# zixunh/vipe

Measured on AMD Instinct MI355X. Metric: dense-BA+flow update iters/s, 512x384 48-KF graph, higher is better.
Workload: dtype f16 (correlation, GRU; fp32 accumulate) + f32 geometry/BA (fp64 reduced system)

## Files before the change

### include/vipe_amd.h

```cpp
#ifndef VIPE_AMD_H
#define VIPE_AMD_H

#include <stdint.h>

#ifdef __cplusplus
extern "C" {
#endif

#define VIPE_F16 0
#define VIPE_F32 1
#define VIPE_F64 2
#define VIPE_U8 3

#define VIPE_OK 0
#define VIPE_EINVAL (-1)
#define VIPE_ENOSPACE (-2)
#define VIPE_EUNSUPPORTED (-3)

#define VIPE_PYRAMID_REFERENCE 0
#define VIPE_PYRAMID_BLOCKED 1

#define VIPE_CAM_PINHOLE 0
#define VIPE_CAM_MEI 1
#define VIPE_CAM_PANORAMA 2

const char* vipe_amd_version(void);
int vipe_amd_abi_version(void);


int vipe_corr_index_forward(const void* d_volume, const float* d_coords, void* d_corr, int B, int h1, int w1,
                            int h2, int w2, int radius, int dtype, void* stream);

int vipe_corr_index_backward(const float* d_coords, const void* d_corr_grad, void* d_volume_grad, int B, int h1,
                             int w1, int h2, int w2, int radius, int dtype, void* stream);

int vipe_corr_pyramid_lookup(const void* const* h_levels, const float* d_coords, void* d_out, int B, int h1, int w1,
                             int h2, int w2, int num_levels, int radius, int dtype, void* stream);

int vipe_corr_pyramid_lookup_nhwc(const void* const* h_levels, const float* d_coords, void* d_out, int B, int h1,
                                  int w1, int h2, int w2, int num_levels, int radius, int dtype, int channel_stride,
                                  void* stream);

int vipe_corr_lookup_conv1x1(const void* const* h_levels, const float* d_coords, const void* d_w_packed,
                             const float* d_bias, void* d_out, int out_ctot, int out_coff, int B, int h1, int w1,
                             int h2, int w2, int Cout, int act, const int* d_slots, int layout, void* stream);

int vipe_corr_pyramid_build(const void* d_fmap1, const void* d_fmap2, void* const* h_levels, int B, int C, int h,
                            int w, int num_levels, void* stream);

int vipe_corr_pyramid_build_indexed(const void* d_fmaps, const int64_t* d_idx1, const int64_t* d_idx2,
                                    const int* d_slots, void* const* h_levels, int B, int C, int h, int w,
                                    int num_levels, int layout, void* stream);

int vipe_corr_blocked_dims(int h, int w, int* dims6);
int64_t vipe_corr_prep_halves(int C, int h, int w);
int vipe_corr_prep(const void* d_fmaps, void* d_prep, int n, int C, int h, int w, void* stream);
int vipe_corr_pyramid_build_prepared(const void* d_prep, int64_t frame_base, int64_t n_prepared, const int64_t* d_idx1, const int64_t* d_idx2,
                                     const int* d_slots, void* const* h_levels, int B, int C, int h, int w, int num_levels,
                                     void* stream);

int vipe_corr_volume(const void* d_fmap1, const void* d_fmap2, void* d_volume, int B, int C, int P, int dtype, void* stream);
int vipe_avg_pool2x2(const void* d_x, void* d_y, int64_t n, int h, int w, int dtype, void* stream);

int vipe_altcorr_forward(const void* d_fmap1, const void* d_fmap2, const float* d_coords, void* d_corr, int B,
                         int H1, int W1, int H2, int W2, int N, int C, int radius, int dtype, void* stream);

int vipe_altcorr_backward(const float* d_fmap1, const float* d_fmap2, const float* d_coords,
                          const float* d_corr_grad, float* d_fmap1_grad, float* d_fmap2_grad, int B, int H1, int W1,
                          int H2, int W2, int N, int C, int radius, void* stream);

int vipe_lie_expm(int group_id, const void* a, void* X, int64_t n, int dtype, int on_device, void* stream);
int vipe_lie_logm(int group_id, const void* X, void* a, int64_t n, int dtype, int on_device, void* stream);
int vipe_lie_inv(int group_id, const void* X, void* Y, int64_t n, int dtype, int on_device, void* stream);
int vipe_lie_mul(int group_id, const void* X, const void* Y, void* Z, int64_t n, int dtype, int on_device,
                 void* stream);
int vipe_lie_adj(int group_id, const void* X, const void* a, void* b, int64_t n, int dtype, int on_device,
                 void* stream);
int vipe_lie_adjT(int group_id, const void* X, const void* a, void* b, int64_t n, int dtype, int on_device,
                  void* stream);
int vipe_lie_act(int group_id, const void* X, const void* p, void* q, int64_t n, int dtype, int on_device,
                 void* stream);
int vipe_lie_act4(int group_id, const void* X, const void* p, void* q, int64_t n, int dtype, int on_device,
                  void* stream);
int vipe_lie_as_matrix(int group_id, const void* X, void* T, int64_t n, int dtype, int on_device,
                       void* stream);
int vipe_lie_projector(int group_id, const void* X, void* P, int64_t n, int dtype, int on_device,
                       void* stream);
int vipe_lie_jinv(int group_id, const void* X, const void* a, void* b, int64_t n, int dtype, int on_device,
                  void* stream);
int vipe_frontend_next_frame(float* d_poses, float* d_disps, int t1, int n_views, int P, int n_mean, int init_pose,
                             void* stream);
int vipe_lie_adjT_bcast(int group_id, const void* X, const void* a, void* b, int64_t n_elem, int64_t rows_per_elem,
                        int dtype, void* stream);
int vipe_lie_act4_bcast(int group_id, const void* X, const void* p, void* q, int64_t n_elem, int64_t rows_per_elem,
                        int dtype, void* stream);
int vipe_lie_expm_backward(int group_id, const void* grad, const void* a, void* da, int64_t n, int dtype,
                           int on_device, void* stream);
int vipe_lie_logm_backward(int group_id, const void* grad, const void* X, void* dX, int64_t n, int dtype,
                           int on_device, void* stream);
int vipe_lie_inv_backward(int group_id, const void* grad, const void* X, void* dX, int64_t n, int dtype,
                          int on_device, void* stream);
int vipe_lie_mul_backward(int group_id, const void* grad, const void* X, const void* Y, void* dX, void* dY,
                          int64_t n, int dtype, int on_device, void* stream);
int vipe_lie_adj_backward(int group_id, const void* grad, const void* X, const void* a, void* dX, void* da,
                          int64_t n, int dtype, int on_device, void* stream);
int vipe_lie_adjT_backward(int group_id, const void* grad, const void* X, const void* a, void* dX, void* da,
                           int64_t n, int dtype, int on_device, void* stream);
int vipe_lie_act_backward(int group_id, const void* grad, const void* X, const void* p, void* dX, void* dp,
                          int64_t n, int dtype, int on_device, void* stream);
int vipe_lie_act4_backward(int group_id, const void* grad, const void* X, const void* p, void* dX, void* dp,
                           int64_t n, int dtype, int on_device, void* stream);


int vipe_reproject(const float* d_poses, const float* d_disps, const float* d_intrinsics, const float* d_rig,
                   const int64_t* d_pi, const int64_t* d_qi, const int64_t* d_pj, const int64_t* d_qj,
                   const int64_t* d_di, float* d_coords, float* d_valid, int M, int ht, int wd, int n_views,
                   int camera, float intr_factor, void* stream);

int vipe_reproject_motion(const float* d_poses, const float* d_disps, const float* d_intrinsics, const float* d_rig,
                          const int64_t* d_pi, const int64_t* d_qi, const int64_t* d_pj, const int64_t* d_qj,
                          const int64_t* d_di, const float* d_target, float* d_coords, void* d_motn, int M, int ht,
                          int wd, int n_views, int camera, float intr_factor, int motn_dtype, void* stream);
int vipe_reproject_motion_nhwc(const float* d_poses, const float* d_disps, const float* d_intrinsics,
                               const float* d_rig, const int64_t* d_pi, const int64_t* d_qi, const int64_t* d_pj,
                               const int64_t* d_qj, const int64_t* d_di, const float* d_target, float* d_coords,
                               void* d_motn, int M, int ht, int wd, int n_views, int camera, float intr_factor,
                               void* stream);

typedef int (*vipe_overlap_fn)(void* user, int piece, int n_pieces, void* stream);

typedef struct {
  int n_poses;
  int n_views;
  int ht, wd;
  int M;
  int t0, t1;
  int n_iters;
  float pose_damping, pose_ep;
  int motion_only;
  int limited_disp;
  int optimize_intrinsics;
  int optimize_rig_rotation;
  int camera;
  float alpha;
  float weight_scale;
  float intr_factor;
  int reuse_plan;
  int path_hint;
  void* overlap_stream;
  vipe_overlap_fn overlap_fn;
  void* overlap_user;
  int solver_options;
  void* profile_ev0;
  void* profile_ev1;
  int profile_iter;
} vipe_ba_params;
#define VIPE_BA_OPT_ONE_CHAIN 1
#define VIPE_BA_OPT_GENERAL_ACCUMULATE 2

int64_t vipe_dense_ba_workspace_bytes(const vipe_ba_params* p);
int vipe_dense_ba(const vipe_ba_params* p, float* d_poses, float* d_disps, const float* d_disps_sens,
                  float* d_intrinsics, float* d_rig, const float* d_target, const float* d_weight,
                  const float* d_disp_damping, const int64_t* d_pi, const int64_t* d_qi, const int64_t* d_pj,
                  const int64_t* d_qj, const int64_t* d_di, void* d_workspace, int64_t workspace_bytes,
                  int* d_info, void* stream);

int vipe_dense_ba_linearize(const vipe_ba_params* p, const float* d_poses, const float* d_disps, const float* d_disps_sens,
                            const float* d_intrinsics, const float* d_rig, const float* d_target, const float* d_weight,
                            const float* d_disp_damping, const int64_t* d_pi, const int64_t* d_qi, const int64_t* d_pj,
                            const int64_t* d_qj, const int64_t* d_di, void* d_workspace, int64_t workspace_bytes,
                            double* d_S_out, int ld_out, int* d_info, void* stream);
int vipe_dense_ba_marginals(const vipe_ba_params* p, void* d_workspace, const double* d_Sinv, int ld, float* d_disp_var,
                            double* d_pose_cov, void* stream);

int64_t vipe_ba_workspace_bytes(int n_poses, int ht, int wd, int E);
int vipe_ba(float* d_poses, float* d_disps, const float* d_intrinsics, const float* d_disps_sens,
            const float* d_targets, const float* d_weights, const float* d_eta, const int64_t* d_ii,
            const int64_t* d_jj, int n_poses, int ht, int wd, int E, int n_eta, int t0, int t1, int iterations,
            float lm, float ep, int motion_only, float* d_dx, float* d_dz, void* d_workspace,
            int64_t workspace_bytes, void* stream);

int vipe_frame_distance(const float* d_poses, const float* d_disps, const float* d_intrinsics, const int64_t* d_pi,
                        const int64_t* d_pj, const int64_t* d_qi, const int64_t* d_qj, const int64_t* d_di,
                        float* d_dist, int M, int ht, int wd, float beta, void* stream);

int vipe_frame_distance_rig(const float* d_poses, const float* d_rig, const float* d_disps, const float* d_intrinsics,
                            int intr_dim, float intr_factor, const int64_t* d_pi, const int64_t* d_qi, const int64_t* d_pj,
                            const int64_t* d_qj, float* d_dist, int M, int n_views, int ht, int wd, float beta,
                            int bidirectional, void* stream);

int vipe_depth_filter(const float* d_poses, const float* d_disps, const float* d_intrinsics, const int64_t* d_inds,
                      const float* d_thresh, float* d_counter, int n, int num, int ht, int wd, void* stream);

int vipe_frame_distance_sphere(const float* d_poses, const float* d_rig, const float* d_disps, const int64_t* d_pi,
                               const int64_t* d_qi, const int64_t* d_pj, const int64_t* d_qj, float* d_dist, int M,
                               int n_views, int ht, int wd, float beta, int bidirectional, void* stream);
int vipe_depth_filter_sphere(const float* d_poses, const float* d_disps, const int64_t* d_inds, const float* d_thresh,
                             float* d_counter, int n, int num, int ht, int wd, void* stream);
int vipe_iproj_sphere(const float* d_poses, const float* d_disps, float* d_points, int n, int ht, int wd, void* stream);

int vipe_projmap(const float* d_poses, const float* d_disps, const float* d_intrinsics, const int64_t* d_ii,
                 const int64_t* d_jj, float* d_coords, float* d_valid, int E, int ht, int wd, void* stream);

int vipe_iproj(const float* d_poses, const float* d_disps, const float* d_intrinsics, float* d_points, int n, int ht,
               int wd, void* stream);

int vipe_scatter(const void* d_src, const int64_t* d_index, void* d_out, int64_t* d_arg_out, int64_t outer,
                 int64_t src_dim, int64_t inner, int64_t out_dim, int reduce, int dtype, void* stream);
int vipe_scatter_rows(const void* d_src, const int64_t* d_index, void* d_out, int64_t* d_arg_out, int64_t outer,
                      int64_t src_dim, int64_t inner, int64_t out_dim, int reduce, int dtype, void* stream);

int vipe_scatter_host(const void* h_src, const int64_t* h_index, void* h_out, int64_t* h_arg_out, int64_t outer,
                      int64_t src_dim, int64_t inner, int64_t out_dim, int reduce, int dtype);

int vipe_scatter_mean_rows_f16(const void* d_src, const int64_t* d_ix, void* d_out, int E, int n_out, int64_t inner,
                               void* stream);

int vipe_segment_mean_nhwc_f16(const void* d_src, int src_ctot, int src_coff, const int* d_order, const int* d_rowptr,
                               void* d_out, int n_out, int64_t rows_per_item, int C, void* stream);

int vipe_corr_sampler_forward(const void* d_in1, const void* d_in2, void* d_out, int B, int C, int H, int W, int kH,
                              int kW, int patchH, int patchW, int padH, int padW, int dilH, int dilW,
                              int dil_patchH, int dil_patchW, int dH, int dW, int dtype, void* stream);
int vipe_corr_sampler_backward(const void* d_in1, const void* d_in2, const void* d_grad_out, void* d_grad1,
                               void* d_grad2, int B, int C, int H, int W, int kH, int kW, int patchH, int patchW,
                               int padH, int padW, int dilH, int dilW, int dil_patchH, int dil_patchW, int dH,
                               int dW, int dtype, void* stream);

int vipe_corr_sampler_forward_host(const float* h_in1, const float* h_in2, float* h_out, int B, int C, int H, int W, int kH,
                                   int kW, int patchH, int patchW, int padH, int padW, int dilH, int dilW, int dil_patchH,
                                   int dil_patchW, int dH, int dW);
int vipe_corr_sampler_backward_host(const float* h_in1, const float* h_in2, const float* h_grad_out, float* h_grad1,
                                    float* h_grad2, int B, int C, int H, int W, int kH, int kW, int patchH, int patchW,
                                    int padH, int padW, int dilH, int dilW, int dil_patchH, int dil_patchW, int dH, int dW);

int vipe_nearest_neighbours(const float* d_query, int qdim, const float* d_tree, int tdim, int64_t M, int64_t N, int knn,
                            float* d_dist, int* d_idx, void* stream);

int vipe_ms_deform_attn_forward(const void* d_value, const int64_t* d_spatial_shapes, const int64_t* d_level_start_index,
                                const void* d_sampling_loc, const void* d_attn_weight, void* d_output, int64_t bs,
                                int64_t Lv, int heads, int C, int L, int64_t Lq, int P, int dtype, void* stream);
int vipe_ms_deform_attn_backward(const void* d_value, const int64_t* d_spatial_shapes, const int64_t* d_level_start_index,
                                 const void* d_sampling_loc, const void* d_attn_weight, const void* d_grad_output,
                                 void* d_grad_value, void* d_grad_sampling_loc, void* d_grad_attn_weight, int64_t bs,
                                 int64_t Lv, int heads, int C, int L, int64_t Lq, int P, int dtype, void* stream);

#define VIPE_ACT_NONE 0
#define VIPE_ACT_RELU 1
#define VIPE_ACT_SIGMOID 2
#define VIPE_ACT_TANH 3
int vipe_conv_pack_weights(const void* d_w_oihw, void* d_w_packed, int Cout, int Cin, int KH, int KW, int src_dtype,
                           void* stream);
int vipe_conv2d_nhwc_f16(const void* d_x, const void* d_w_packed, const float* d_bias, const float* d_extra,
                         void* d_y, int B, int H, int W, int Cin, int cin_total, int cin_off, int Cout,
                         int cout_total, int cout_off, int KH, int KW, int act, void* stream);

int vipe_conv_packed_dims(int Cout, int Cin, int KH, int KW, int* cout_pad, int* cin_pad, int* k_pad);

#define VIPE_CONV_PARTIAL 6
#define VIPE_CONV_ACCINIT_F32 0x100
int vipe_conv2d_fused(const void* d_x0, int x0_ctot, int x0_coff, const void* d_x1, int x1_ctot, int x1_coff,
                      int split, const void* d_w_packed, const float* d_bias, const float* d_extra, int extra_stride,
                      int extra_off, void* d_y, int y_ctot, int y_coff, void* d_y2, int y2_ctot, int y2_coff,
                      const void* d_net, int net_ctot, int net_coff, const void* d_z, float* d_fout,
                      const void* d_accinit, int ai_ctot, int ai_coff, int B, int H, int W, int Cin, int Cout, int KH,
                      int KW, int act, int mode, void* stream);

typedef struct {
  const void *corr0_w, *corr2_w, *flow0_w, *flow2_w, *gw_w, *zr_w, *q_w, *zr_s_w, *q_s_w, *heads0_w, *heads2_w, *agg2_w, *eta_w;
  const void *zr_n_w, *zr_x_w;
  const float *corr0_b, *corr2_b, *flow0_b, *flow2_b, *gw_b, *zr_b, *q_b, *heads0_b, *heads2_b, *agg2_b, *eta_b;
  const float* glo_wT;
  const float* glo_b;
} vipe_update_weights;
typedef struct {
  int E, H, W, n_src;
  const void* levels[4];
  const float* coords;
  const int* slots;
  int h2, w2, pyramid_layout;
  const void* corr;
  const void* motn;
  const void* net;
  void* net_out;
  void* xbuf;
  const void* pgate;
  void *c1, *f1, *zb, *rnet;
  void* hbuf;
  float* dw;
  float *glo, *extra;
  const int *order, *rowptr;
  void *agg, *a2;
  float* eta;
  void* side_stream;
  float* pzr;
  int gate_state;
} vipe_update_buffers;
int vipe_update_operator(const vipe_update_weights* weights, const vipe_update_buffers* buffers, void* stream);

int vipe_update_gate_state(const vipe_update_weights* weights, const vipe_update_buffers* buffers, const void* d_net,
                           int parts, void* stream);
typedef struct {
  const vipe_update_weights* weights;
  const vipe_update_buffers* buffers;
  const void* net;
  const int* bounds;
  int n_bounds;
} vipe_gate_state_job;
int vipe_update_gate_state_piece(void* user, int piece, int n_pieces, void* stream);

int vipe_glo_context(const float* d_glo_sum, const float* d_wT, const float* d_bias, float* d_extra, int E, int hw,
                     void* stream);

typedef struct {
  const void* src;
  void* dst;
  const int64_t* idx;
  int64_t src_row_pitch, dst_row_pitch;
  int64_t seg_bytes, seg_pitch;
  int n_seg;
  int n_rows;
  int dst_row0;
} vipe_rows_job;
int vipe_rows_gather(const vipe_rows_job* jobs, int n_jobs, void* stream);
typedef struct {
  const void* src;
  const int64_t* frame;
  void* dst;
  int64_t dst_row_pitch;
  int dst_ctot, dst_coff;
  int dst_row0;
} vipe_nhwc_job;
int vipe_gather_nchw_to_nhwc_f16(const vipe_nhwc_job* jobs, int n_jobs, int n_rows, int C, int P, void* stream);

int vipe_flow_score(const float* d_dw, const unsigned char* d_invalid, float* d_score, int n_views, int P, void* stream);

int vipe_update_finish(const float* d_coords1, const float* d_dw, const unsigned char* d_mask, float* d_target,
                       float* d_weight, const float* d_eta, const int64_t* d_du, float* d_damping, int E, int n_src, int ht,
                       int wd, void* stream);

int vipe_enc_prep(const float* d_img, void* d_x4, int V, int H, int W, void* stream);
int vipe_enc_stem(const void* d_x4, const void* d_w, const float* d_bias, void* d_y, float* d_out_stats, int B, int H,
                  int W, int relu, void* stream);
int vipe_enc_conv(const void* d_x, const float* d_in_stats, const void* d_w, const float* d_bias, const void* d_res,
                  void* d_y, float* d_out_stats, int B, int H, int W, int Cin, int Cout, int ksize, int stride,
                  int relu, int nchw, int tanh_split, void* stream);
int vipe_enc_finish(const void* d_raw, const float* d_raw_stats, const void* d_res, const float* d_res_stats,
                    void* d_out, int B, int HW, int C, void* stream);

int vipe_frame_ingest(const void* d_rgb, int rgb_dtype, const unsigned char* d_mask, const float* d_depth, int H0, int W0,
                      int h1, int w1, int top, int left, int H, int W, float* d_images, void* d_x4,
                      unsigned char* d_mask8, float* d_disps_sens, void* stream);

int vipe_convex_upsample(const void* d_mask, int mask_dtype, const float* d_data, float* d_out, const int64_t* d_rows,
                         int N, int R, int h, int w, int C, void* stream);

#define VIPE_KLT_OOB 1
#define VIPE_KLT_LOW_TEXTURE 2
#define VIPE_KLT_RESIDUAL 4
#define VIPE_KLT_FB 8
#define VIPE_KLT_MASKED 16
#define VIPE_KLT_DIVERGED 32

int vipe_klt_pyramid(const void* d_rgb, int rgb_dtype, int H, int W, int L, float* d_pyr, void* stream);

int vipe_klt_detect(const float* d_img, int H, int W, const unsigned char* d_mask, const unsigned char* d_cell_busy,
                    int cell, int border, float min_eig, float* d_out, void* stream);

int vipe_klt_track(const float* d_pyr_a, const float* d_pyr_b, int H, int W, int L, const float* d_pts, int N,
                   const float* d_fb_ref, const unsigned char* d_mask, int win_radius, int n_iters, float eps, int border,
                   float min_eig, float max_residual, float fb_thresh, float max_flow, int cell, float* d_out,
                   unsigned char* d_status, float* d_resid, unsigned char* d_cell_busy, void* stream);

#ifdef __cplusplus
}
#endif
#endif
```

### vipe_amd/csrc/conv_mfma.hip

```cpp
#include <stdlib.h>

#include <type_traits>

#include "common.cuh"

namespace {

typedef _Float16 half8 __attribute__((ext_vector_type(8)));
typedef _Float16 half4 __attribute__((ext_vector_type(4)));
typedef float float16v __attribute__((ext_vector_type(16)));
typedef float float4v __attribute__((ext_vector_type(4)));

enum Epi { EPI_PLAIN = 0, EPI_GLO = 1, EPI_ZR = 2, EPI_Q = 3, EPI_HEADS = 4, EPI_ETA = 5, EPI_PARTIAL = 6 };

struct ConvArgs {
  const half_t* x0; int x0_ctot, x0_coff;
  const half_t* x1; int x1_ctot, x1_coff;
  int split;
  const half_t* w;
  const float* bias;
  const float* extra;
  int extra_stride, extra_off;
  half_t* y; int y_ctot, y_coff;
  int B, H, W, Cin, Cin_pad, Cout, Cout_pad, KH, KW, nsteps;
  int act, epi;
  const half_t* net; int net_ctot, net_coff;
  const half_t* zbuf;
  half_t* y2; int y2_ctot, y2_coff;
  float* fout;
  const half_t* accinit; int ai_ctot, ai_coff;
  int ai_f32;
  int f_wp, f_hwp, f_tiles, f_pieces, f_xbytes, f_p1lo, f_p1hi;
  unsigned f_magic;
};

constexpr int BNP = 128;
constexpr int BK = 64;

__device__ __forceinline__ int swz(int row, int k8) { return row * 128 + ((k8 ^ ((row >> 1) & 7)) << 4); }

__device__ __forceinline__ float act_apply(float v, int act) {
  switch (act) {
    case VIPE_ACT_RELU: return fmaxf(v, 0.0f);
    case VIPE_ACT_SIGMOID: return 1.0f / (1.0f + __expf(-v));
    case VIPE_ACT_TANH: return tanhf(v);
    default: return v;
  }
}

template <int BMC, int WAVES_M, int WAVES_N, bool SMALLCIN>
__global__ __launch_bounds__(256) void conv_mfma_kernel(ConvArgs a) {
  constexpr int TM = BMC / (WAVES_M * 32);
  constexpr int TN = BNP / (WAVES_N * 32);
  static_assert(WAVES_M * WAVES_N == 4, "4 waves");
  constexpr int W_ITEMS = BMC * 8 / 256;
  constexpr int X_ITEMS = BNP * 8 / 256;

  extern __shared__ __align__(16) unsigned char lds[];
  unsigned char* ldsW = lds;
  unsigned char* ldsX = lds + 2 * BMC * 128;

  const int tid = threadIdx.x, lane = tid & 63, wave = tid >> 6;
  const int wm = wave / WAVES_N, wn = wave % WAVES_N;
  const int64_t M = (int64_t)a.B * a.H * a.W;
  const int64_t pix0 = (int64_t)blockIdx.x * BNP;
  const int cout0 = blockIdx.y * BMC;
  const int HW = a.H * a.W;

  const int k8 = tid & 7;
  int xe[X_ITEMS], xy[X_ITEMS], xx[X_ITEMS];
  bool xvalid[X_ITEMS];
#pragma unroll
  for (int j = 0; j < X_ITEMS; ++j) {
    const int64_t m = pix0 + (tid >> 3) + 32 * j;
    xvalid[j] = m < M;
    const int64_t mm = xvalid[j] ? m : 0;
    xe[j] = (int)(mm / HW);
    const int rem = (int)(mm % HW);
    xy[j] = rem / a.W;
    xx[j] = rem % a.W;
  }
  const int ph = a.KH / 2, pw = a.KW / 2;
  const int csteps = a.Cin_pad / BK;

  half8 wreg[W_ITEMS], xreg[X_ITEMS];

  auto issue_loads = [&](int s) {
    const half_t* wb = a.w + ((int64_t)s * a.Cout_pad + cout0) * BK;
#pragma unroll
    for (int j = 0; j < W_ITEMS; ++j) {
      const int row = (tid >> 3) + 32 * j;
      wreg[j] = *reinterpret_cast<const half8*>(wb + row * BK + k8 * 8);
    }
    if constexpr (!SMALLCIN) {
      const int tap = s / csteps, c0 = (s % csteps) * BK;
      const int dy = tap / a.KW - ph, dx = tap % a.KW - pw;
      const int c = c0 + k8 * 8;
      const bool cok = c < a.Cin;
      const bool s0 = c < a.split;
      const half_t* src = s0 ? a.x0 : a.x1;
      const int ctot = s0 ? a.x0_ctot : a.x1_ctot;
      const int coff = s0 ? a.x0_coff + c : a.x1_coff + (c - a.split);
#pragma unroll
      for (int j = 0; j < X_ITEMS; ++j) {
        const int yy = xy[j] + dy, xc = xx[j] + dx;
        const bool ok = cok & xvalid[j] & (yy >= 0) & (yy < a.H) & (xc >= 0) & (xc < a.W);
        half8 v = {0, 0, 0, 0, 0, 0, 0, 0};
        if (ok) v = *reinterpret_cast<const half8*>(src + ((int64_t)(xe[j] * a.H + yy) * a.W + xc) * ctot + coff);
        xreg[j] = v;
      }
    } else {
      const int q = s * 8 + k8;
#pragma unroll
      for (int j = 0; j < X_ITEMS; ++j) {
        half4 lo = {0, 0, 0, 0}, hi = {0, 0, 0, 0};
#pragma unroll
        for (int h = 0; h < 2; ++h) {
          const int tap = 2 * q + h;
          if (tap < a.KH * a.KW) {
            const int yy = xy[j] + tap / a.KW - ph, xc = xx[j] + tap % a.KW - pw;
            if (xvalid[j] & (yy >= 0) & (yy < a.H) & (xc >= 0) & (xc < a.W)) {
              const half4 v = *reinterpret_cast<const half4*>(
                  a.x0 + ((int64_t)(xe[j] * a.H + yy) * a.W + xc) * a.x0_ctot + a.x0_coff);
              if (h == 0) lo = v; else hi = v;
            }
          }
        }
        xreg[j] = half8{lo[0], lo[1], lo[2], lo[3], hi[0], hi[1], hi[2], hi[3]};
      }
    }
  };
  auto write_lds = [&](int buf) {
#pragma unroll
    for (int j = 0; j < W_ITEMS; ++j) {
      const int row = (tid >> 3) + 32 * j;
      *reinterpret_cast<half8*>(ldsW + buf * BMC * 128 + swz(row, k8)) = wreg[j];
    }
#pragma unroll
    for (int j = 0; j < X_ITEMS; ++j) {
      const int row = (tid >> 3) + 32 * j;
      *reinterpret_cast<half8*>(ldsX + buf * BNP * 128 + swz(row, k8)) = xreg[j];
    }
  };

  float16v acc[TM][TN];
#pragma unroll
  for (int i = 0; i < TM; ++i)
#pragma unroll
    for (int j = 0; j < TN; ++j)
#pragma unroll
      for (int r = 0; r < 16; ++r) acc[i][j][r] = 0.0f;

  issue_loads(0);
  write_lds(0);
  __syncthreads();
  const int lrow = lane & 31, lhalf = lane >> 5;
  for (int s = 0; s < a.nsteps; ++s) {
    const int cur = s & 1;
    if (s + 1 < a.nsteps) issue_loads(s + 1);
    const unsigned char* bw = ldsW + cur * BMC * 128;
    const unsigned char* bx = ldsX + cur * BNP * 128;
#pragma unroll
    for (int kk = 0; kk < BK / 16; ++kk) {
      half8 wf[TM], xf[TN];
#pragma unroll
      for (int i = 0; i < TM; ++i)
        wf[i] = *reinterpret_cast<const half8*>(bw + swz((wm * TM + i) * 32 + lrow, kk * 2 + lhalf));
#pragma unroll
      for (int j = 0; j < TN; ++j)
        xf[j] = *reinterpret_cast<const half8*>(bx + swz((wn * TN + j) * 32 + lrow, kk * 2 + lhalf));
#pragma unroll
      for (int i = 0; i < TM; ++i)
#pragma unroll
        for (int j = 0; j < TN; ++j)
          acc[i][j] = __builtin_amdgcn_mfma_f32_32x32x16_f16(wf[i], xf[j], acc[i][j], 0, 0, 0);
    }
    if (s + 1 < a.nsteps) write_lds(cur ^ 1);
    __syncthreads();
  }

#include "conv_epilogue.inc"
}

__device__ __attribute__((aligned(16))) unsigned char g_zero_page[64];

__device__ __forceinline__ void glds16(const void* g, unsigned lds_addr) {
#if defined(__HIP_DEVICE_COMPILE__)
  unsigned keep;
  const unsigned base = __builtin_amdgcn_readfirstlane(lds_addr);
  asm volatile(
      "s_mov_b32 %0, m0\n\ts_mov_b32 m0, %2\n\ts_nop 0\n\tglobal_load_lds_dwordx4 %1, off\n\ts_mov_b32 m0, %0"
      : "=&s"(keep)
      : "v"(g), "s"(base)
      : "memory");
#endif
}

__device__ __forceinline__ unsigned lds_address(const void* p) {
  return (unsigned)(uintptr_t)(__attribute__((address_space(3))) const unsigned char*)p;
}

template <int BMC, int WAVES_M, int WAVES_N>
__global__ __launch_bounds__(256) void conv_mfma_glds_kernel(ConvArgs a, int gy) {
  constexpr int TM = BMC / (WAVES_M * 32);
  constexpr int TN = BNP / (WAVES_N * 32);
  static_assert(WAVES_M * WAVES_N == 4, "4 waves");
  constexpr int WP = BMC / 32;
  constexpr int XP = BNP / 32;

  extern __shared__ __align__(16) unsigned char lds[];
  unsigned char* ldsW = lds;
  unsigned char* ldsX = lds + 2 * BMC * 128;

  const int tid = threadIdx.x, lane = tid & 63, wave = __builtin_amdgcn_readfirstlane(tid >> 6);
  const int wm = wave / WAVES_N, wn = wave % WAVES_N;
  const int nb = gridDim.x;
  const int L = xcd_remap(blockIdx.x, nb);
  const int64_t M = (int64_t)a.B * a.H * a.W;
  const int64_t pix0 = (int64_t)(L / gy) * BNP;
  const int cout0 = (L % gy) * BMC;
  const int HW = a.H * a.W;
  const int ph = a.KH / 2, pw = a.KW / 2;
  const int csteps = a.Cin_pad / BK;
  const int r8 = lane >> 3, sl = lane & 7;

  int woff[WP];
#pragma unroll
  for (int q = 0; q < WP; ++q) {
    const int row = (wave * WP + q) * 8 + r8;
    woff[q] = row * BK + ((sl ^ ((row >> 1) & 7)) << 3);
  }
  const half_t* xb0[XP];
  const half_t* xb1[XP];
  int xk8[XP], py[XP], px[XP];
  unsigned xmask[XP];
#pragma unroll
  for (int q = 0; q < XP; ++q) {
    const int row = (wave * XP + q) * 8 + r8;
    const int64_t m = pix0 + row;
    const bool ok = m < M;
    const int64_t mm = ok ? m : 0;
    const int rem = (int)(mm % HW);
    py[q] = ok ? rem / a.W : -100000;
    px[q] = rem % a.W;
    const int k8 = sl ^ ((row >> 1) & 7);
    xk8[q] = k8 * 8;
    xb0[q] = a.x0 + mm * a.x0_ctot + a.x0_coff + k8 * 8;
    xb1[q] = a.x1 + mm * a.x1_ctot + a.x1_coff + k8 * 8 - a.split;
    xmask[q] = 0;
  }
  for (int t = 0; t < a.KH * a.KW; ++t) {
    const int dy = t / a.KW - ph, dx = t % a.KW - pw;
#pragma unroll
    for (int q = 0; q < XP; ++q) {
      const int yy = py[q] + dy, xc = px[q] + dx;
      if (yy >= 0 && yy < a.H && xc >= 0 && xc < a.W) xmask[q] |= 1u << t;
    }
  }
  const half_t* zp = reinterpret_cast<const half_t*>(g_zero_page);

  auto issue = [&](int s, int buf) {
    const half_t* wb = a.w + ((int64_t)s * a.Cout_pad + cout0) * BK;
    unsigned char* lw = ldsW + buf * BMC * 128 + wave * WP * 1024;
#pragma unroll
    for (int q = 0; q < WP; ++q)
      glds16(wb + woff[q], lds_address(lw) + q * 1024);
    const int tap = s / csteps, c0 = (s % csteps) * BK;
    const int dy = tap / a.KW - ph, dx = tap % a.KW - pw;
    const bool s0 = c0 < a.split;
    const int64_t delta = (int64_t)(dy * a.W + dx) * (s0 ? a.x0_ctot : a.x1_ctot) + c0;
    const int crem = a.Cin - c0;
    unsigned char* lx = ldsX + buf * BNP * 128 + wave * XP * 1024;
#pragma unroll
    for (int q = 0; q < XP; ++q) {
      const bool ok = ((xmask[q] >> tap) & 1u) && (xk8[q] < crem);
      const half_t* p = (s0 ? xb0[q] : xb1[q]) + delta;
      glds16(ok ? p : zp, lds_address(lx) + q * 1024);
    }
  };

  float16v acc[TM][TN];
#pragma unroll
  for (int i = 0; i < TM; ++i)
#pragma unroll
    for (int j = 0; j < TN; ++j)
#pragma unroll
      for (int r = 0; r < 16; ++r) acc[i][j][r] = 0.0f;

  issue(0, 0);
  asm volatile("s_waitcnt vmcnt(0)" ::: "memory");
  __syncthreads();
  const int lrow = lane & 31, lhalf = lane >> 5;
  for (int s = 0; s < a.nsteps; ++s) {
    const int cur = s & 1;
    const unsigned char* bw = ldsW + cur * BMC * 128;
    const unsigned char* bx = ldsX + cur * BNP * 128;
    half8 wf[BK / 16][TM], xf[BK / 16][TN];
#pragma unroll
    for (int kk = 0; kk < BK / 16; ++kk) {
#pragma unroll
      for (int i = 0; i < TM; ++i)
        wf[kk][i] = *reinterpret_cast<const half8*>(bw + swz((wm * TM + i) * 32 + lrow, kk * 2 + lhalf));
#pragma unroll
      for (int j = 0; j < TN; ++j)
        xf[kk][j] = *reinterpret_cast<const half8*>(bx + swz((wn * TN + j) * 32 + lrow, kk * 2 + lhalf));
    }
    __builtin_amdgcn_sched_barrier(0);
    if (s + 1 < a.nsteps) issue(s + 1, cur ^ 1);
    __builtin_amdgcn_sched_barrier(0);
#pragma unroll
    for (int kk = 0; kk < BK / 16; ++kk)
#pragma unroll
      for (int i = 0; i < TM; ++i)
#pragma unroll
        for (int j = 0; j < TN; ++j)
          acc[i][j] = __builtin_amdgcn_mfma_f32_32x32x16_f16(wf[kk][i], xf[kk][j], acc[i][j], 0, 0, 0);
    asm volatile("s_waitcnt vmcnt(0)" ::: "memory");
    __syncthreads();
  }
#include "conv_epilogue.inc"
}

constexpr int HALO_TH = 4, HALO_TW = 64;
constexpr int HALO_PITCH = HALO_TW + 2;
constexpr int HALO_ROWS = (HALO_TH + 2) * HALO_PITCH;

__device__ __forceinline__ void glds16_off(const void* base, unsigned voff_bytes, unsigned lds_addr) {
#if defined(__HIP_DEVICE_COMPILE__)
  unsigned keep;
  const unsigned lb = __builtin_amdgcn_readfirstlane(lds_addr);
  const uint64_t bu = (uint64_t)base;
  const uint64_t bs = ((uint64_t)(unsigned)__builtin_amdgcn_readfirstlane((int)(bu >> 32)) << 32) |
                      (unsigned)__builtin_amdgcn_readfirstlane((int)bu);
  asm volatile(
      "s_mov_b32 %0, m0\n\ts_mov_b32 m0, %3\n\ts_nop 0\n\tglobal_load_lds_dwordx4 %1, %2\n\ts_mov_b32 m0, %0"
      : "=&s"(keep)
      : "v"(voff_bytes), "s"(bs), "s"(lb)
      : "memory");
#endif
}

__device__ __forceinline__ uint64_t uniform64(uint64_t v) {
  return ((uint64_t)(unsigned)__builtin_amdgcn_readfirstlane((int)(v >> 32)) << 32) | (unsigned)__builtin_amdgcn_readfirstlane((int)v);
}
__device__ __forceinline__ void dma16s(uint64_t sbase, unsigned voff_bytes, unsigned lds_addr) {
#if defined(__HIP_DEVICE_COMPILE__)
  unsigned keep;
  asm volatile("s_mov_b32 %0, m0\n\ts_mov_b32 m0, %3\n\ts_nop 0\n\tglobal_load_lds_dwordx4 %1, %2\n\ts_mov_b32 m0, %0"
               : "=&s"(keep)
               : "v"(voff_bytes), "s"(sbase), "s"(lds_addr)
               : "memory");
#endif
}
__device__ __forceinline__ void dma16v(uint64_t lane_ptr, unsigned lds_addr) {
#if defined(__HIP_DEVICE_COMPILE__)
  unsigned keep;
  asm volatile("s_mov_b32 %0, m0\n\ts_mov_b32 m0, %2\n\ts_nop 0\n\tglobal_load_lds_dwordx4 %1, off\n\ts_mov_b32 m0, %0"
               : "=&s"(keep)
               : "v"(lane_ptr), "s"(lds_addr)
               : "memory");
#endif
}

constexpr int H32_PIECES = (HALO_ROWS + 15) / 16;
constexpr int H32_XBYTES = H32_PIECES * 1024;
constexpr int H32_XP = (H32_PIECES + 7) / 8;
constexpr int H32_BK = 32;

__device__ __forceinline__ int swzf(int row) { return ((row >> 2) & 1) << 1; }
__device__ __forceinline__ int swz32(int row, int c) { return row * 64 + ((c ^ swzf(row)) << 4); }


__device__ __forceinline__ int flat_pixel(int q, int e, int H, int W, int wp, int hwp, unsigned magic) {
  if ((unsigned)q >= (unsigned)hwp) return -1;
  const int y = (int)__umulhi((unsigned)q, magic);
  const int x = q - y * wp;
  return x < W ? (e * H + y) * W + x : -1;
}

template <int BMC, int KS, bool M16, int VAR = 0, bool FLAT = false>
__global__ __launch_bounds__(512) __attribute__((amdgpu_waves_per_eu(4, 4))) void conv_halo32_kernel(ConvArgs a, int gy) {
  static_assert(M16, "only the 16x16x32 form exists");
  constexpr int MI = BMC >= 128 ? 4 : 2, NJ = BMC == 32 ? 2 : 4;
  constexpr int BP = HALO_TH * HALO_TW;
  constexpr int WSTAGE = BMC * 64;
  extern __shared__ __align__(16) unsigned char lds[];

  const int tid = threadIdx.x, lane = tid & 63, wave = __builtin_amdgcn_readfirstlane(tid >> 6);
  const int wm = BMC == 32 ? 0 : (wave >> 2), wn = wave & 3;
  const int pxh = BMC == 32 ? (wave >> 2) * 32 : 0;
  const int L = xcd_remap(blockIdx.x, gridDim.x);
  const int tile = L / gy, cout0 = (L % gy) * BMC;
  const int xsegs = a.W / HALO_TW, tiles_per_img = FLAT ? a.f_tiles : (a.H / HALO_TH) * xsegs;
  const int e = tile / tiles_per_img, trem = tile % tiles_per_img;
  const int y0 = (trem / xsegs) * HALO_TH, x0 = (trem % xsegs) * HALO_TW;
  const int q0 = trem * BP;
  const int pitch = FLAT ? a.f_wp : HALO_PITCH;
  const int xbytes = FLAT ? a.f_xbytes : H32_XBYTES;
  const int npieces = FLAT ? a.f_pieces : H32_PIECES;
  auto pix_of = [&](int pl) -> int64_t {
    if constexpr (FLAT) return flat_pixel(q0 + pl, e, a.H, a.W, a.f_wp, a.f_hwp, a.f_magic);
    else return ((int64_t)(e * a.H + y0 + (pl >> 6))) * a.W + x0 + (pl & 63);
  };
  const int cs32 = a.Cin_pad / H32_BK, cs64 = a.Cin_pad / 64;
  const int r16 = lane >> 2, sl = lane & 3;

  const unsigned ldsW_a = lds_address(lds), ldsX_a = ldsW_a + 3 * WSTAGE;
  const unsigned sink_a = ldsX_a + 2 * xbytes;
  const unsigned char* ldsW = lds;
  const unsigned char* ldsX = lds + 3 * WSTAGE;
  const half_t* zp = reinterpret_cast<const half_t*>(g_zero_page);

  constexpr int WPIECES = BMC / 16;
  const bool wreal = wave < WPIECES;
  const int wrow = (wave % WPIECES) * 16 + r16;
  const unsigned woff = (unsigned)(wrow * 64 + ((sl ^ swzf(wrow)) << 3)) * 2u;
  const unsigned wdst = ldsW_a + (wave % WPIECES) * 1024;
  int xpix[FLAT ? 1 : H32_XP];
  const int xk = (sl ^ swzf(r16)) * 8;
  if constexpr (!FLAT) {
#pragma unroll
    for (int i = 0; i < H32_XP; ++i) {
      const int pce = wave + 8 * i;
      const int r = pce * 16 + r16;
      const int hy = r / HALO_PITCH, hx = r % HALO_PITCH;
      const int y = y0 + hy - 1, x = x0 + hx - 1;
      const bool ok = pce < H32_PIECES && r < HALO_ROWS && y >= 0 && y < a.H && x >= 0 && x < a.W;
      xpix[i] = ok ? (e * a.H + y) * a.W + x : -1;
    }
  }
  auto piece_used = [&](int i) {
    const int pce = wave + 8 * i;
    if constexpr (FLAT) return pce < npieces && (KS == 3 || (pce >= a.f_p1lo && pce <= a.f_p1hi));
    else return pce < H32_PIECES && (KS == 3 || (pce >= 4 && pce <= 20));
  };
  auto issueX = [&](int c, int i, int buf) {
    const int c0 = c * H32_BK;
    const bool s0 = c0 < a.split;
    const int ctot = s0 ? a.x0_ctot : a.x1_ctot;
    const int cb = (s0 ? a.x0_coff : a.x1_coff - a.split) + c0;
    int xp;
    if constexpr (FLAT) xp = flat_pixel(q0 - pitch - 1 + (wave + 8 * i) * 16 + r16, e, a.H, a.W, a.f_wp, a.f_hwp, a.f_magic);
    else xp = xpix[i];
    const bool ok = xp >= 0 && (c0 + xk < a.Cin);
    const uint64_t off = ((uint64_t)(unsigned)xp * (unsigned)ctot + (unsigned)(cb + xk)) * 2u;
    const char* src = reinterpret_cast<const char*>(s0 ? a.x0 : a.x1) + off;
    glds16(ok ? (const void*)src : (const void*)zp, ldsX_a + buf * xbytes + (wave + 8 * i) * 1024);
  };
  auto wsrc = [&](int tap, int c) {
    return a.w + ((int64_t)(tap * cs64 + (c >> 1)) * a.Cout_pad + cout0) * BK + (c & 1) * H32_BK;
  };
  auto issueW = [&](const half_t* wb, int slot) {
    if (wreal) glds16_off(wb, woff, wdst + slot * WSTAGE);
    else glds16(zp, sink_a);
  };
  const uint64_t zp64 = uniform64((uint64_t)zp);
  const uint64_t wbase = uniform64((uint64_t)(a.w + (int64_t)cout0 * BK));
  const unsigned tstride = (unsigned)cs64 * (unsigned)a.Cout_pad * BK * 2u;
  const unsigned sink_u = __builtin_amdgcn_readfirstlane(sink_a), wdst_u = __builtin_amdgcn_readfirstlane(wdst);
  const unsigned ldsX_u = __builtin_amdgcn_readfirstlane(ldsX_a + wave * 1024);
  auto issueW2 = [&](int tap, int c, int slot, bool more_) {
    const unsigned off = (unsigned)tap * tstride + ((unsigned)(c >> 1) * (unsigned)a.Cout_pad * BK + (unsigned)(c & 1) * H32_BK) * 2u;
    const bool on = more_ && wreal;
    dma16s(on ? wbase + off : zp64, on ? woff : 0u, on ? wdst_u + slot * WSTAGE : sink_u);
  };
  auto issueX2 = [&](int c, int i, int buf, bool on) {
    const int c0 = c * H32_BK;
    const bool s0 = c0 < a.split;
    const int ctot = s0 ? a.x0_ctot : a.x1_ctot;
    const int cb = (s0 ? a.x0_coff : a.x1_coff - a.split) + c0;
    int xp;
    if constexpr (FLAT) xp = flat_pixel(q0 - pitch - 1 + (wave + 8 * i) * 16 + r16, e, a.H, a.W, a.f_wp, a.f_hwp, a.f_magic);
    else xp = xpix[i];
    const bool ok = on && xp >= 0 && (c0 + xk < a.Cin);
    const uint64_t off = ((uint64_t)(unsigned)xp * (unsigned)ctot + (unsigned)(cb + xk)) * 2u;
    const uint64_t base = (uint64_t)(s0 ? a.x0 : a.x1);
    dma16v(ok ? base + off : zp64, on ? ldsX_u + buf * xbytes + i * 8192 : sink_u);
  };

  float4v acc16[MI][NJ];
#pragma unroll
  for (int i = 0; i < MI; ++i)
#pragma unroll
    for (int j = 0; j < NJ; ++j) acc16[i][j] = float4v{0.0f, 0.0f, 0.0f, 0.0f};
  if constexpr (BMC >= 64) {
    if (a.accinit) {
#pragma unroll
      for (int j = 0; j < NJ; ++j) {
        const int64_t m = pix_of(wn * 64 + j * 16 + (lane & 15));
        if (FLAT && m < 0) continue;
#pragma unroll
        for (int i = 0; i < MI; ++i) {
          const int cg = cout0 + wm * (MI * 16) + i * 16 + 4 * (lane >> 4);
          if constexpr (VAR == 1) {
            const float4 v = *reinterpret_cast<const float4*>(reinterpret_cast<const float*>(a.accinit) + m * a.ai_ctot +
                                                              a.ai_coff + cg);
            acc16[i][j] = float4v{v.x, v.y, v.z, v.w};
          } else {
            const half4 v = *reinterpret_cast<const half4*>(a.accinit + m * a.ai_ctot + a.ai_coff + cg);
            acc16[i][j] = float4v{(float)v[0], (float)v[1], (float)v[2], (float)v[3]};
          }
        }
      }
    }
  }

  const int l16 = lane & 15, lk = lane >> 4;
  const int wa0 = swz32(wm * MI * 16 + l16, lk);
  const int Rl0 = (FLAT ? wn * HALO_TW : wn * HALO_PITCH) + pxh + l16;
  auto mma_step = [&](const unsigned char* bw, const unsigned char* bx, int Rl, int dy, int dx) {
    const int rb = Rl + (dy + 1) * pitch + (dx + 1);
    const int xa0 = swz32(rb, lk);
    half8 wf[MI];
#pragma unroll
    for (int i = 0; i < MI; ++i) wf[i] = *reinterpret_cast<const half8*>(bw + (wa0 + i * 1024));
#pragma unroll
    for (int j = 0; j < NJ; ++j) {
      const half8 xf = *reinterpret_cast<const half8*>(bx + (xa0 + j * 1024));
#pragma unroll
      for (int i = 0; i < MI; ++i)
        acc16[i][j] = __builtin_amdgcn_mfma_f32_16x16x32_f16(wf[i], xf, acc16[i][j], 0, 0, 0);
    }
  };

  auto load_frags = [&](const unsigned char* bw, const unsigned char* bx, int Rl, int dy, int dx, half8 (&wf)[MI], half8 (&xf)[NJ]) {
    const int xa0 = swz32(Rl + (dy + 1) * pitch + (dx + 1), lk);
#pragma unroll
    for (int i = 0; i < MI; ++i) wf[i] = *reinterpret_cast<const half8*>(bw + (wa0 + i * 1024));
#pragma unroll
    for (int j = 0; j < NJ; ++j) xf[j] = *reinterpret_cast<const half8*>(bx + (xa0 + j * 1024));
  };
  auto mma_frags = [&](const half8 (&wf)[MI], const half8 (&xf)[NJ]) {
#pragma unroll
    for (int j = 0; j < NJ; ++j)
#pragma unroll
      for (int i = 0; i < MI; ++i) acc16[i][j] = __builtin_amdgcn_mfma_f32_16x16x32_f16(wf[i], xf[j], acc16[i][j], 0, 0, 0);
  };

#pragma unroll
  for (int i = 0; i < H32_XP; ++i)
    if (piece_used(i)) issueX(0, i, 0);
  issueW(wsrc(0, 0), 0);
  if constexpr (KS == 3) issueW(wsrc(1, 0), 1);
  asm volatile("s_waitcnt vmcnt(0)" ::: "memory");
  __syncthreads();

  if constexpr (KS == 3) {
    for (int c = 0; c < cs32; ++c) {
      const unsigned char* bx = ldsX + (c & 1) * xbytes;
      const bool more = c + 1 < cs32;
      int Rl = Rl0;
      asm volatile("" : "+v"(Rl));
      auto tap_step = [&](auto TAPC) {
        constexpr int TAP = decltype(TAPC)::value;
        constexpr int T2 = TAP + 2;
        half8 wf[MI], xf[NJ];
        load_frags(ldsW + (TAP % 3) * WSTAGE, bx, Rl, TAP / 3 - 1, TAP % 3 - 1, wf, xf);
        if constexpr (T2 < 9) issueW2(T2, c, T2 % 3, true);
        else issueW2(T2 - 9, c + 1, T2 % 3, more);
        if constexpr (TAP < H32_XP) issueX2(c + 1, TAP, (c + 1) & 1, more && piece_used(TAP));
        mma_frags(wf, xf);
        if constexpr (TAP == 0 || TAP == 4) asm volatile("s_waitcnt vmcnt(2)" ::: "memory");
        else if constexpr (TAP < 4) asm volatile("s_waitcnt vmcnt(3)" ::: "memory");
        else asm volatile("s_waitcnt vmcnt(1)" ::: "memory");
        __syncthreads();
      };
      tap_step(std::integral_constant<int, 0>{});
      tap_step(std::integral_constant<int, 1>{});
      tap_step(std::integral_constant<int, 2>{});
      tap_step(std::integral_constant<int, 3>{});
      tap_step(std::integral_constant<int, 4>{});
      tap_step(std::integral_constant<int, 5>{});
      tap_step(std::integral_constant<int, 6>{});
      tap_step(std::integral_constant<int, 7>{});
      tap_step(std::integral_constant<int, 8>{});
    }
  } else {
    for (int c = 0; c < cs32; ++c) {
      const unsigned char* bx = ldsX + (c & 1) * xbytes;
      if (c + 1 < cs32) {
        issueW(wsrc(0, c + 1), (c + 1) & 1);
#pragma unroll
        for (int i = 0; i < H32_XP; ++i)
          if (piece_used(i)) issueX(c + 1, i, (c + 1) & 1);
      }
      mma_step(ldsW + (c & 1) * WSTAGE, bx, Rl0, 0, 0);
      asm volatile("s_waitcnt vmcnt(0)" ::: "memory");
      __syncthreads();
    }
  }
  asm volatile("s_waitcnt vmcnt(0)" ::: "memory");
  __syncthreads();

  constexpr int CPP = BMC / 8;
  constexpr int NIT = BP * CPP / 512, PSTEP = 512 / CPP;
  const int ch = (tid % CPP) * 8, co = cout0 + ch, pl0 = tid / CPP;
  if constexpr (BMC >= 64) {
    if constexpr (VAR == 2) {
      {
#pragma unroll
        for (int j = 0; j < NJ; ++j) {
          const int64_t m = pix_of(wn * 64 + j * 16 + l16);
          if (FLAT && m < 0) continue;
#pragma unroll
          for (int i = 0; i < MI; ++i) {
            const int cg = cout0 + wm * (MI * 16) + i * 16 + 4 * lk;
            if (cg + 4 <= a.Cout)
              *reinterpret_cast<float4*>(a.fout + m * a.y_ctot + a.y_coff + cg) =
                  make_float4(acc16[i][j][0], acc16[i][j][1], acc16[i][j][2], acc16[i][j][3]);
          }
        }
        return;
      }
    }
    constexpr int PITCH = BMC + 8;
    half_t* stage = reinterpret_cast<half_t*>(lds);
    auto stage_all = [&](auto ACTC) {
      constexpr int ACT = decltype(ACTC)::value;
      auto put = [&](int cl, int pl, float4 b, float v0, float v1, float v2, float v3) {
        half4 h;
        h[0] = (half_t)act_apply(v0 + b.x, ACT);
        h[1] = (half_t)act_apply(v1 + b.y, ACT);
        h[2] = (half_t)act_apply(v2 + b.z, ACT);
        h[3] = (half_t)act_apply(v3 + b.w, ACT);
        *reinterpret_cast<half4*>(stage + pl * PITCH + cl) = h;
      };
      auto bias4 = [&](int cl) {
        const int cg = cout0 + cl;
        float4 b = *reinterpret_cast<const float4*>(a.bias + cg);
        if (a.extra && cg + 4 <= a.Cout) {
          const float4 x = *reinterpret_cast<const float4*>(a.extra + (int64_t)e * a.extra_stride + a.extra_off + cg);
          b.x += x.x; b.y += x.y; b.z += x.z; b.w += x.w;
        }
        return b;
      };
#pragma unroll
      for (int i = 0; i < MI; ++i) {
        const int cl = wm * (MI * 16) + i * 16 + 4 * lk;
        const float4 b = bias4(cl);
#pragma unroll
        for (int j = 0; j < NJ; ++j)
          put(cl, wn * 64 + j * 16 + l16, b, acc16[i][j][0], acc16[i][j][1], acc16[i][j][2], acc16[i][j][3]);
      }
    };
    const int actsel = a.epi == EPI_PLAIN ? a.act : (a.epi == EPI_Q ? VIPE_ACT_TANH : VIPE_ACT_SIGMOID);
    if (actsel == VIPE_ACT_RELU) stage_all(std::integral_constant<int, VIPE_ACT_RELU>{});
    else if (actsel == VIPE_ACT_SIGMOID) stage_all(std::integral_constant<int, VIPE_ACT_SIGMOID>{});
    else if (actsel == VIPE_ACT_TANH) stage_all(std::integral_constant<int, VIPE_ACT_TANH>{});
    else stage_all(std::integral_constant<int, VIPE_ACT_NONE>{});
    const bool want_net = a.epi == EPI_GLO || a.epi == EPI_Q || (a.epi == EPI_ZR && co >= 128);
    const bool want_z = a.epi == EPI_Q;
    half8 nvv[NIT], zvv[NIT];
    {
      const int cn = a.epi == EPI_ZR ? co - 128 : co;
#pragma unroll
      for (int it = 0; it < NIT; ++it) {
        const int64_t m = pix_of(pl0 + PSTEP * it);
        if (FLAT && m < 0) continue;
        if (want_net) nvv[it] = *reinterpret_cast<const half8*>(a.net + m * a.net_ctot + a.net_coff + cn);
        if (want_z) zvv[it] = *reinterpret_cast<const half8*>(a.zbuf + m * 128 + co);
      }
    }
    __syncthreads();
    float gsum[8] = {0, 0, 0, 0, 0, 0, 0, 0};
#pragma unroll
    for (int it = 0; it < NIT; ++it) {
      const int pl = pl0 + PSTEP * it;
      const int64_t m = pix_of(pl);
      if (FLAT && m < 0) continue;
      const half8 sv = *reinterpret_cast<const half8*>(stage + pl * PITCH + ch);
      half8 o = sv;
      half_t* dst = nullptr;
      if (a.epi == EPI_PLAIN) {
        dst = a.y + m * a.y_ctot + a.y_coff + co;
      } else if (a.epi == EPI_GLO) {
#pragma unroll
        for (int q = 0; q < 8; ++q) gsum[q] += (float)sv[q] * (float)nvv[it][q];
      } else if (a.epi == EPI_ZR) {
        if (co < 128) {
          dst = a.y + m * a.y_ctot + a.y_coff + co;
        } else {
#pragma unroll
          for (int q = 0; q < 8; ++q) o[q] = (half_t)((float)sv[q] * (float)nvv[it][q]);
          dst = a.y2 + m * a.y2_ctot + a.y2_coff + co - 128;
        }
      } else if (a.epi == EPI_Q) {
#pragma unroll
        for (int q = 0; q < 8; ++q) {
          const float z = (float)zvv[it][q];
          o[q] = (half_t)((1.0f - z) * (float)nvv[it][q] + z * (float)sv[q]);
        }
        dst = a.y + m * a.y_ctot + a.y_coff + co;
      }
      if (dst) {
        if (co + 8 <= a.Cout) {
          *reinterpret_cast<half8*>(dst) = o;
        } else {
          for (int q = 0; q < 8 && co + q < a.Cout; ++q) dst[q] = o[q];
        }
      }
    }
    if (a.epi == EPI_GLO) {
      float* red = reinterpret_cast<float*>(lds);
      __syncthreads();
#pragma unroll
      for (int q = 0; q < 8; ++q) red[(tid / CPP) * (BMC + 1) + ch + q] = gsum[q];
      __syncthreads();
      if (tid < BMC) {
        float t = 0.0f;
        for (int r = 0; r < 512 / CPP; ++r) t += red[r * (BMC + 1) + tid];
        if (cout0 + tid < a.Cout) atomicAdd(a.fout + (int64_t)e * a.Cout + cout0 + tid, t);
      }
    }
  } else {
    constexpr int PITCH = BMC + 4;
    float* stage = reinterpret_cast<float*>(lds);
#pragma unroll
    for (int i = 0; i < MI; ++i)
#pragma unroll
      for (int j = 0; j < NJ; ++j)
        *reinterpret_cast<float4*>(stage + (wn * 64 + pxh + j * 16 + l16) * PITCH + i * 16 + 4 * lk) =
            make_float4(acc16[i][j][0], acc16[i][j][1], acc16[i][j][2], acc16[i][j][3]);
    __syncthreads();
    float bv[8];
#pragma unroll
    for (int q = 0; q < 8; ++q) {
      bv[q] = a.bias[co + q];
      if (a.extra && co + q < a.Cout) bv[q] += a.extra[(int64_t)e * a.extra_stride + a.extra_off + co + q];
    }
#pragma unroll
    for (int it = 0; it < NIT; ++it) {
      const int pl = pl0 + PSTEP * it;
      const int64_t m = pix_of(pl);
      if (FLAT && m < 0) continue;
      const float4 v0 = *reinterpret_cast<const float4*>(stage + pl * PITCH + ch);
      const float4 v1 = *reinterpret_cast<const float4*>(stage + pl * PITCH + ch + 4);
      const float v[8] = {v0.x + bv[0], v0.y + bv[1], v0.z + bv[2], v0.w + bv[3],
                          v1.x + bv[4], v1.y + bv[5], v1.z + bv[6], v1.w + bv[7]};
      if (a.epi == EPI_HEADS) {
        if (ch == 0)
          *reinterpret_cast<float4*>(a.fout + m * 4) =
              make_float4((float)(half_t)v[0], (float)(half_t)v[1], (float)(half_t)act_apply(v[2], VIPE_ACT_SIGMOID),
                          (float)(half_t)act_apply(v[3], VIPE_ACT_SIGMOID));
      } else if (a.epi == EPI_ETA) {
        if (ch == 0) {
          const float sp = v[0] > 20.0f ? v[0] : log1pf(__expf(v[0]));
          a.fout[m] = 0.01f * (float)(half_t)sp;
        }
      } else {
        half_t* dst = a.y + m * a.y_ctot + a.y_coff + co;
        half8 o;
#pragma unroll
        for (int q = 0; q < 8; ++q) o[q] = (half_t)act_apply(v[q], a.act);
        if (co + 8 <= a.Cout) {
          *reinterpret_cast<half8*>(dst) = o;
        } else {
          for (int q = 0; q < 8 && co + q < a.Cout; ++q) dst[q] = o[q];
        }
      }
    }
  }
}

constexpr int NRW_WBYTES = 9 * 1024;

template <bool FLAT>
__global__ __launch_bounds__(512) __attribute__((amdgpu_waves_per_eu(4, 4))) void conv_halo32_narrow_kernel(ConvArgs a) {
  extern __shared__ __align__(16) unsigned char lds[];
  const int tid = threadIdx.x, lane = tid & 63, wave = __builtin_amdgcn_readfirstlane(tid >> 6);
  const int wn = wave & 3, pxh = (wave >> 2) * 32;
  const int tile = xcd_remap(blockIdx.x, gridDim.x);
  const int xsegs = a.W / HALO_TW, tiles_per_img = FLAT ? a.f_tiles : (a.H / HALO_TH) * xsegs;
  const int e = tile / tiles_per_img, trem = tile % tiles_per_img;
  const int y0 = (trem / xsegs) * HALO_TH, x0 = (trem % xsegs) * HALO_TW;
  const int q0 = trem * (HALO_TH * HALO_TW);
  const int pitch = FLAT ? a.f_wp : HALO_PITCH, xbytes = FLAT ? a.f_xbytes : H32_XBYTES;
  const int npieces = FLAT ? a.f_pieces : H32_PIECES;
  auto pix_of = [&](int pl) -> int64_t {
    if constexpr (FLAT) return flat_pixel(q0 + pl, e, a.H, a.W, a.f_wp, a.f_hwp, a.f_magic);
    else return ((int64_t)(e * a.H + y0 + (pl >> 6))) * a.W + x0 + (pl & 63);
  };
  const int cs32 = a.Cin_pad / H32_BK, cs64 = a.Cin_pad / 64;
  const int r16 = lane >> 2, sl = lane & 3, l16 = lane & 15, lk = lane >> 4;
  const unsigned ldsW_a = lds_address(lds), ldsX_a = ldsW_a + 2 * NRW_WBYTES;
  const unsigned char* ldsW = lds;
  const unsigned char* ldsX = lds + 2 * NRW_WBYTES;
  const half_t* zp = reinterpret_cast<const half_t*>(g_zero_page);

  int xpix[H32_XP];
  const int xk = (sl ^ swzf(r16)) * 8;
#pragma unroll
  for (int i = 0; i < H32_XP; ++i) {
    const int pce = wave + 8 * i;
    const int r = pce * 16 + r16;
    if constexpr (FLAT) {
      xpix[i] = pce < npieces ? flat_pixel(q0 - pitch - 1 + r, e, a.H, a.W, a.f_wp, a.f_hwp, a.f_magic) : -1;
    } else {
      const int hy = r / HALO_PITCH, hx = r % HALO_PITCH;
      const int y = y0 + hy - 1, x = x0 + hx - 1;
      const bool ok = pce < H32_PIECES && r < HALO_ROWS && y >= 0 && y < a.H && x >= 0 && x < a.W;
      xpix[i] = ok ? (e * a.H + y) * a.W + x : -1;
    }
  }
  auto issue = [&](int c, int buf) {
    const int c0 = c * H32_BK;
    const bool s0 = c0 < a.split;
    const int ctot = s0 ? a.x0_ctot : a.x1_ctot;
    const int cb = (s0 ? a.x0_coff : a.x1_coff - a.split) + c0;
#pragma unroll
    for (int i = 0; i < H32_XP; ++i) {
      if (wave + 8 * i < npieces) {
        const bool ok = xpix[i] >= 0 && (c0 + xk < a.Cin);
        const uint64_t off = ((uint64_t)(unsigned)xpix[i] * (unsigned)ctot + (unsigned)(cb + xk)) * 2u;
        const char* src = reinterpret_cast<const char*>(s0 ? a.x0 : a.x1) + off;
        glds16(ok ? (const void*)src : (const void*)zp, ldsX_a + buf * xbytes + (wave + 8 * i) * 1024);
      }
    }
    const unsigned woff = (unsigned)(r16 * 64 + ((sl ^ swzf(r16)) << 3)) * 2u;
    const half_t* wb = a.w + ((int64_t)(wave * cs64 + (c >> 1)) * a.Cout_pad) * BK + (c & 1) * H32_BK;
    glds16_off(wb, woff, ldsW_a + buf * NRW_WBYTES + wave * 1024);
    if (wave == 0) {
      const half_t* w8 = a.w + ((int64_t)(8 * cs64 + (c >> 1)) * a.Cout_pad) * BK + (c & 1) * H32_BK;
      glds16_off(w8, woff, ldsW_a + buf * NRW_WBYTES + 8 * 1024);
    }
  };

  float4v acc[2] = {float4v{0.f, 0.f, 0.f, 0.f}, float4v{0.f, 0.f, 0.f, 0.f}};
  const int wa0 = swz32(l16, lk);
  const int Rl0 = (FLAT ? wn * HALO_TW : wn * HALO_PITCH) + pxh + l16;
  issue(0, 0);
  asm volatile("s_waitcnt vmcnt(0)" ::: "memory");
  __syncthreads();
  for (int c = 0; c < cs32; ++c) {
    if (c + 1 < cs32) issue(c + 1, (c + 1) & 1);
    const unsigned char* bw = ldsW + (c & 1) * NRW_WBYTES;
    const unsigned char* bx = ldsX + (c & 1) * xbytes;
#pragma unroll
    for (int tap = 0; tap < 9; ++tap) {
      const int rb = Rl0 + (tap / 3) * pitch + (tap % 3);
      const int xa0 = swz32(rb, lk);
      const half8 wf = *reinterpret_cast<const half8*>(bw + (wa0 + tap * 1024));
#pragma unroll
      for (int j = 0; j < 2; ++j) {
        const half8 xf = *reinterpret_cast<const half8*>(bx + (xa0 + j * 1024));
        acc[j] = __builtin_amdgcn_mfma_f32_16x16x32_f16(wf, xf, acc[j], 0, 0, 0);
      }
    }
    asm volatile("s_waitcnt vmcnt(0)" ::: "memory");
    __syncthreads();
  }
  constexpr int PITCH = 20;
  float* stage = reinterpret_cast<float*>(lds);
#pragma unroll
  for (int j = 0; j < 2; ++j)
    *reinterpret_cast<float4*>(stage + (wn * 64 + pxh + j * 16 + l16) * PITCH + 4 * lk) =
        make_float4(acc[j][0], acc[j][1], acc[j][2], acc[j][3]);
  __syncthreads();
  const int64_t m = tid < HALO_TH * HALO_TW ? pix_of(tid) : -1;
  if (tid < HALO_TH * HALO_TW && (!FLAT || m >= 0)) {
    float v[16];
#pragma unroll
    for (int q = 0; q < 4; ++q) {
      const float4 t4 = *reinterpret_cast<const float4*>(stage + tid * PITCH + 4 * q);
      v[4 * q] = t4.x; v[4 * q + 1] = t4.y; v[4 * q + 2] = t4.z; v[4 * q + 3] = t4.w;
    }
#pragma unroll
    for (int q = 0; q < 16; ++q) {
      v[q] += a.bias[q];
      if (a.extra && q < a.Cout) v[q] += a.extra[(int64_t)e * a.extra_stride + a.extra_off + q];
    }
    if (a.epi == EPI_HEADS) {
      *reinterpret_cast<float4*>(a.fout + m * 4) =
          make_float4((float)(half_t)v[0], (float)(half_t)v[1], (float)(half_t)act_apply(v[2], VIPE_ACT_SIGMOID),
                      (float)(half_t)act_apply(v[3], VIPE_ACT_SIGMOID));
    } else if (a.epi == EPI_ETA) {
      const float sp = v[0] > 20.0f ? v[0] : log1pf(__expf(v[0]));
      a.fout[m] = 0.01f * (float)(half_t)sp;
    } else {
      half_t* dst = a.y + m * a.y_ctot + a.y_coff;
      for (int q = 0; q < a.Cout; ++q) dst[q] = (half_t)act_apply(v[q], a.act);
    }
  }
}

constexpr int GLO_PITCH = 136;
constexpr size_t GLO_LDS = 256 * GLO_PITCH * 2 + 128 * 4;

__global__ __launch_bounds__(512) __attribute__((amdgpu_waves_per_eu(4, 4))) void conv1x1_glo_kernel(ConvArgs a) {
  extern __shared__ __align__(16) unsigned char lds[];
  half_t* xt = reinterpret_cast<half_t*>(lds);
  float* gacc = reinterpret_cast<float*>(lds + 256 * GLO_PITCH * 2);
  const int tid = threadIdx.x, lane = tid & 63, wave = tid >> 6;
  const int l16 = lane & 15, kg = lane >> 4;
  const int wq = wave & 3, wp = wave >> 2;
  const int HW = a.H * a.W;
  const int tpi = (HW + 255) / 256;
  const int e = blockIdx.x / tpi, p0 = (blockIdx.x % tpi) * 256;
  const int64_t pix0 = (int64_t)e * HW + p0;
  if (tid < 128) gacc[tid] = 0.0f;
#pragma unroll
  for (int it = 0; it < 8; ++it) {
    const int i = tid + 512 * it, px = i >> 4, ck = i & 15;
    half8 v = {0, 0, 0, 0, 0, 0, 0, 0};
    if (p0 + px < HW) v = *reinterpret_cast<const half8*>(a.x0 + (pix0 + px) * a.x0_ctot + a.x0_coff + ck * 8);
    *reinterpret_cast<half8*>(xt + px * GLO_PITCH + ck * 8) = v;
  }
  half8 af[2][4];
#pragma unroll
  for (int i = 0; i < 2; ++i)
#pragma unroll
    for (int s2 = 0; s2 < 4; ++s2) {
      const int k = 32 * s2 + 8 * kg, r = 32 * wq + 16 * i + l16;
      af[i][s2] = *reinterpret_cast<const half8*>(a.w + ((int64_t)(k >> 6) * a.Cout_pad + r) * 64 + (k & 63));
    }
  float4 bv[2];
#pragma unroll
  for (int i = 0; i < 2; ++i) bv[i] = *reinterpret_cast<const float4*>(a.bias + 32 * wq + 16 * i + 4 * kg);
  __syncthreads();
  float gs[2][4] = {{0, 0, 0, 0}, {0, 0, 0, 0}};
#pragma unroll 2
  for (int j = 0; j < 8; ++j) {
    const int pxb = wp * 128 + j * 16 + l16;
    float4v acc[2] = {float4v{0.f, 0.f, 0.f, 0.f}, float4v{0.f, 0.f, 0.f, 0.f}};
#pragma unroll
    for (int s2 = 0; s2 < 4; ++s2) {
      const half8 xf = *reinterpret_cast<const half8*>(xt + pxb * GLO_PITCH + 32 * s2 + 8 * kg);
#pragma unroll
      for (int i = 0; i < 2; ++i) acc[i] = __builtin_amdgcn_mfma_f32_16x16x32_f16(af[i][s2], xf, acc[i], 0, 0, 0);
    }
#pragma unroll
    for (int i = 0; i < 2; ++i) {
      const half4 nv = *reinterpret_cast<const half4*>(xt + pxb * GLO_PITCH + 32 * wq + 16 * i + 4 * kg);
      const float b4[4] = {bv[i].x, bv[i].y, bv[i].z, bv[i].w};
#pragma unroll
      for (int r = 0; r < 4; ++r)
        gs[i][r] += (float)(half_t)act_apply(acc[i][r] + b4[r], VIPE_ACT_SIGMOID) * (float)nv[r];
    }
  }
#pragma unroll
  for (int i = 0; i < 2; ++i)
#pragma unroll
    for (int r = 0; r < 4; ++r) {
      float v = gs[i][r];
      v += __builtin_bit_cast(float, __builtin_amdgcn_update_dpp(0, __builtin_bit_cast(int, v), 0xB1, 0xf, 0xf, true));
      v += __builtin_bit_cast(float, __builtin_amdgcn_update_dpp(0, __builtin_bit_cast(int, v), 0x4E, 0xf, 0xf, true));
      v += __builtin_bit_cast(float, __builtin_amdgcn_update_dpp(0, __builtin_bit_cast(int, v), 0x141, 0xf, 0xf, true));
      v += __builtin_bit_cast(float, __builtin_amdgcn_update_dpp(0, __builtin_bit_cast(int, v), 0x140, 0xf, 0xf, true));
      if (l16 == 0) atomicAdd(&gacc[32 * wq + 16 * i + 4 * kg + r], v);
    }
  __syncthreads();
  if (tid < a.Cout) atomicAdd(a.fout + (int64_t)e * a.Cout + tid, gacc[tid]);
}

constexpr int C7_PW = HALO_TW + 6, C7_ROWS = HALO_TH + 6;
constexpr int C7_WBYTES = 4 * 128 * 128;
constexpr int C7_XBYTES = ((C7_PW * C7_ROWS * 8 + 15) / 16) * 16;
constexpr int C7_LDS = (C7_WBYTES + C7_XBYTES) > (256 * 136 * 2) ? (C7_WBYTES + C7_XBYTES) : (256 * 136 * 2);

template <bool FLAT>
__global__ __launch_bounds__(512) __attribute__((amdgpu_waves_per_eu(4, 4))) void conv7x7_c4_kernel(ConvArgs a, int gy) {
  extern __shared__ __align__(16) unsigned char lds[];
  const int tid = threadIdx.x, lane = tid & 63, wave = __builtin_amdgcn_readfirstlane(tid >> 6);
  const int wm = wave >> 2, wn = wave & 3;
  const int L = xcd_remap(blockIdx.x, gridDim.x);
  const int tile = L / gy, cout0 = (L % gy) * 128;
  const int xsegs = a.W / HALO_TW, tiles_per_img = FLAT ? a.f_tiles : (a.H / HALO_TH) * xsegs;
  const int e = tile / tiles_per_img, trem = tile % tiles_per_img;
  const int y0 = (trem / xsegs) * HALO_TH, x0 = (trem % xsegs) * HALO_TW;
  const int q0 = trem * (HALO_TH * HALO_TW), pitch = FLAT ? a.f_wp : C7_PW;
  auto pix_of = [&](int pl) -> int64_t {
    if constexpr (FLAT) return flat_pixel(q0 + pl, e, a.H, a.W, a.f_wp, a.f_hwp, a.f_magic);
    else return ((int64_t)(e * a.H + y0 + (pl >> 6))) * a.W + x0 + (pl & 63);
  };
  const int l16 = lane & 15, lk = lane >> 4;
  const unsigned ldsW_a = lds_address(lds);
  unsigned char* ldsX = lds + C7_WBYTES;

  {
    const int r8 = lane >> 3, sl = lane & 7;
#pragma unroll
    for (int q = 0; q < 8; ++q) {
      const int pce = wave * 8 + q;
      const int blk = pce >> 4, row = (pce & 15) * 8 + r8;
      const half_t* src = a.w + ((int64_t)blk * a.Cout_pad + cout0 + row) * 64 + ((sl ^ ((row >> 1) & 7)) << 3);
      glds16(src, ldsW_a + pce * 1024);
    }
  }
  if constexpr (FLAT) {
    const int nh = HALO_TH * HALO_TW + 6 * pitch + 6;
    for (int i = tid; i < nh; i += 512) {
      const int m = flat_pixel(q0 - 3 * pitch - 3 + i, e, a.H, a.W, a.f_wp, a.f_hwp, a.f_magic);
      uint2 v = make_uint2(0u, 0u);
      if (m >= 0) v = *reinterpret_cast<const uint2*>(a.x0 + (int64_t)m * a.x0_ctot + a.x0_coff);
      *reinterpret_cast<uint2*>(ldsX + i * 8) = v;
    }
  } else {
    for (int i = tid; i < C7_PW * C7_ROWS; i += 512) {
      const int hy = i / C7_PW, hx = i % C7_PW;
      const int y = y0 + hy - 3, x = x0 + hx - 3;
      uint2 v = make_uint2(0u, 0u);
      if (y >= 0 && y < a.H && x >= 0 && x < a.W)
        v = *reinterpret_cast<const uint2*>(a.x0 + ((int64_t)(e * a.H + y) * a.W + x) * a.x0_ctot + a.x0_coff);
      *reinterpret_cast<uint2*>(ldsX + i * 8) = v;
    }
  }
  asm volatile("s_waitcnt vmcnt(0)" ::: "memory");
  __syncthreads();

  float4v acc[4][4];
#pragma unroll
  for (int i = 0; i < 4; ++i)
#pragma unroll
    for (int j = 0; j < 4; ++j) acc[i][j] = float4v{0.0f, 0.0f, 0.0f, 0.0f};
#pragma unroll
  for (int st = 0; st < 7; ++st) {
    half8 wf[4];
#pragma unroll
    for (int i = 0; i < 4; ++i)
      wf[i] = *reinterpret_cast<const half8*>(lds + (st >> 1) * 16384 + swz(wm * 64 + i * 16 + l16, (st & 1) * 4 + lk));
    const int t0 = min(st * 8 + lk * 2, 48), t1 = min(st * 8 + lk * 2 + 1, 48);
    const int wrow = FLAT ? wn * HALO_TW : wn * C7_PW;
    const int o0 = (wrow + (t0 / 7) * pitch + l16 + t0 % 7) * 8, o1 = (wrow + (t1 / 7) * pitch + l16 + t1 % 7) * 8;
#pragma unroll
    for (int j = 0; j < 4; ++j) {
      const half4 lo = *reinterpret_cast<const half4*>(ldsX + o0 + j * 128);
      const half4 hi = *reinterpret_cast<const half4*>(ldsX + o1 + j * 128);
      const half8 xf = {lo[0], lo[1], lo[2], lo[3], hi[0], hi[1], hi[2], hi[3]};
#pragma unroll
      for (int i = 0; i < 4; ++i) acc[i][j] = __builtin_amdgcn_mfma_f32_16x16x32_f16(wf[i], xf, acc[i][j], 0, 0, 0);
    }
  }
  __syncthreads();
  constexpr int PITCH = 136;
  half_t* stage = reinterpret_cast<half_t*>(lds);
#pragma unroll
  for (int i = 0; i < 4; ++i) {
    const int cl = wm * 64 + i * 16 + 4 * lk;
    const float4 b = *reinterpret_cast<const float4*>(a.bias + cout0 + cl);
#pragma unroll
    for (int j = 0; j < 4; ++j) {
      half4 h;
      h[0] = (half_t)act_apply(acc[i][j][0] + b.x, a.act);
      h[1] = (half_t)act_apply(acc[i][j][1] + b.y, a.act);
      h[2] = (half_t)act_apply(acc[i][j][2] + b.z, a.act);
      h[3] = (half_t)act_apply(acc[i][j][3] + b.w, a.act);
      *reinterpret_cast<half4*>(stage + (wn * 64 + j * 16 + l16) * PITCH + cl) = h;
    }
  }
  __syncthreads();
  const int ch = (tid & 15) * 8, co = cout0 + ch;
#pragma unroll
  for (int it = 0; it < 8; ++it) {
    const int pl = (tid >> 4) + 32 * it;
    const int64_t m = pix_of(pl);
    if (FLAT && m < 0) continue;
    const half8 o = *reinterpret_cast<const half8*>(stage + pl * PITCH + ch);
    half_t* dst = a.y + m * a.y_ctot + a.y_coff + co;
    if (co + 8 <= a.Cout) {
      *reinterpret_cast<half8*>(dst) = o;
    } else {
      for (int q = 0; q < 8 && co + q < a.Cout; ++q) dst[q] = o[q];
    }
  }
}

__global__ void pack_weights_kernel(const void* __restrict__ src, half_t* __restrict__ dst, int Cout, int Cin, int KH,
                                    int KW, int Cout_pad, int Cin_pad, int K_pad, int src_f32, int smallcin) {
  const int64_t total = (int64_t)K_pad * Cout_pad;
  for (int64_t i = (int64_t)blockIdx.x * blockDim.x + threadIdx.x; i < total; i += (int64_t)gridDim.x * blockDim.x) {
    const int kin = (int)(i % 64);
    const int co = (int)((i / 64) % Cout_pad);
    const int s = (int)(i / (64 * (int64_t)Cout_pad));
    const int k = s * 64 + kin;
    int tap, c;
    if (smallcin) { tap = k / 4; c = k % 4; }
    else { tap = k / Cin_pad; c = k % Cin_pad; }
    float v = 0.0f;
    if (co < Cout && c < Cin && tap < KH * KW) {
      const int64_t o = (((int64_t)co * Cin + c) * KH + tap / KW) * KW + tap % KW;
      v = src_f32 ? reinterpret_cast<const float*>(src)[o] : (float)reinterpret_cast<const half_t*>(src)[o];
    }
    dst[i] = (half_t)v;
  }
}

inline int round_up(int x, int m) { return (x + m - 1) / m * m; }

}


extern "C" {

VIPE_EXPORT int vipe_conv_packed_dims(int Cout, int Cin, int KH, int KW, int* cout_pad, int* cin_pad, int* k_pad) {
  if (Cout <= 0 || Cin <= 0 || KH <= 0 || KW <= 0) return VIPE_EINVAL;
  const int cp = Cout <= 32 ? 32 : (Cout <= 64 ? 64 : round_up(Cout, 128));
  int cinp, kp;
  if (Cin == 4) { cinp = 4; kp = round_up(KH * KW * 4, 64); }
  else { cinp = round_up(Cin, 64); kp = KH * KW * cinp; }
  if (cout_pad) *cout_pad = cp;
  if (cin_pad) *cin_pad = cinp;
  if (k_pad) *k_pad = kp;
  return VIPE_OK;
}

VIPE_EXPORT int vipe_conv_pack_weights(const void* d_w_oihw, void* d_w_packed, int Cout, int Cin, int KH, int KW,
                                       int src_dtype, void* stream) {
  VIPE_CHECK_ARG(d_w_oihw && d_w_packed);
  VIPE_CHECK_ARG(src_dtype == VIPE_F16 || src_dtype == VIPE_F32);
  int cp, cinp, kp;
  if (vipe_conv_packed_dims(Cout, Cin, KH, KW, &cp, &cinp, &kp) != VIPE_OK) return VIPE_EINVAL;
  VIPE_CHECK_ARG(Cin == 4 || Cin % 8 == 0);
  const int64_t total = (int64_t)kp * cp;
  pack_weights_kernel<<<(int)std::min<int64_t>((total + 255) / 256, 4096), 256, 0, as_stream(stream)>>>(
      d_w_oihw, (half_t*)d_w_packed, Cout, Cin, KH, KW, cp, cinp, kp, src_dtype == VIPE_F32, Cin == 4);
  return vipe_launch_status();
}

}

namespace {

template <typename K>
void allow_lds(K kernel, std::atomic<uint64_t>& seen, size_t bytes) {
  vipe_once_per_device(seen, [&] { (void)hipFuncSetAttribute((const void*)kernel, hipFuncAttributeMaxDynamicSharedMemorySize, (int)bytes); });
}
constexpr size_t MAX_LDS = 160 * 1024;

bool flat_geometry(ConvArgs& a, int pad) {
  a.f_wp = a.W + pad;
  a.f_hwp = a.H * a.f_wp;
  a.f_tiles = (a.f_hwp + 255) / 256;
  a.f_magic = (unsigned)(((1ull << 32) + (unsigned)a.f_wp - 1) / (unsigned)a.f_wp);
  const int rows = 256 + 2 * a.f_wp + 2;
  a.f_pieces = (rows + 15) / 16;
  a.f_xbytes = a.f_pieces * 1024;
  a.f_p1lo = (a.f_wp + 1) / 16;
  a.f_p1hi = (a.f_wp + 256) / 16;
  return a.f_wp >= 2 && a.f_pieces <= 8 * H32_XP && a.f_hwp < (1 << 23);
}

inline bool needs_tile_kernel(const ConvArgs& a) { return a.accinit || a.epi == EPI_PARTIAL || a.ai_f32; }

template <int BMC, int KS, int VAR, bool FLAT>
int launch_halo32(const ConvArgs& a, int tiles, int gy, size_t lds, hipStream_t s) {
  static std::atomic<uint64_t> seen{0};
  allow_lds(conv_halo32_kernel<BMC, KS, true, VAR, FLAT>, seen, FLAT ? MAX_LDS : lds);
  conv_halo32_kernel<BMC, KS, true, VAR, FLAT><<<dim3(tiles * gy), 512, lds, s>>>(a, gy);
  return vipe_launch_status();
}

template <bool FLAT>
int launch_halo_family(ConvArgs& a, int cp, int64_t M, hipStream_t s) {
  const bool split_ok = a.split >= a.Cin || a.split % H32_BK == 0;
  const int tiles = FLAT ? a.B * a.f_tiles : (int)(M / (HALO_TH * HALO_TW));
  const size_t xb = FLAT ? (size_t)a.f_xbytes : (size_t)H32_XBYTES;
  if (needs_tile_kernel(a)) {
    const bool ok = cp >= 64 && split_ok && !(a.KH == 3 && a.Cout <= 16) && !(a.epi == EPI_PARTIAL && a.Cout % 4 != 0) &&
                    !(a.ai_f32 && !a.accinit);
    if (!ok) return VIPE_EUNSUPPORTED;
  }
  if (a.KH == 3 && a.Cout <= 16 && cp == 32 && split_ok && (a.epi == EPI_HEADS || a.epi == EPI_ETA || a.epi == EPI_PLAIN)) {
    static std::atomic<uint64_t> seen{0};
    const size_t lds = 2 * NRW_WBYTES + 2 * xb + 1024;
    allow_lds(conv_halo32_narrow_kernel<FLAT>, seen, FLAT ? MAX_LDS : lds);
    conv_halo32_narrow_kernel<FLAT><<<dim3(tiles), 512, lds, s>>>(a);
    return vipe_launch_status();
  }
  if (!split_ok) return VIPE_EUNSUPPORTED;
  const int bmc = cp >= 128 ? 128 : cp;
  const int gy = cp >= 128 ? cp / 128 : 1;
  size_t lds = 3 * (size_t)bmc * 64 + 2 * xb + 1024;
  const size_t stage = bmc >= 64 ? (size_t)256 * (bmc + 8) * 2 : (size_t)256 * 36 * 4;
  if (lds < stage) lds = stage;
  if (a.ai_f32 || a.epi == EPI_PARTIAL) {
    if (!(a.KH == 3 && bmc == 128 && !(a.ai_f32 && a.epi == EPI_PARTIAL))) return VIPE_EUNSUPPORTED;
    return a.ai_f32 ? launch_halo32<128, 3, 1, FLAT>(a, tiles, gy, lds, s) : launch_halo32<128, 3, 2, FLAT>(a, tiles, gy, lds, s);
  }
  if (a.KH == 3) {
    if (bmc == 128) return launch_halo32<128, 3, 0, FLAT>(a, tiles, gy, lds, s);
    if (bmc == 64) return launch_halo32<64, 3, 0, FLAT>(a, tiles, 1, lds, s);
    return launch_halo32<32, 3, 0, FLAT>(a, tiles, 1, lds, s);
  }
  if (bmc == 128) return launch_halo32<128, 1, 0, FLAT>(a, tiles, gy, lds, s);
  if (bmc == 64) return launch_halo32<64, 1, 0, FLAT>(a, tiles, 1, lds, s);
  return launch_halo32<32, 1, 0, FLAT>(a, tiles, 1, lds, s);
}

int launch_conv(ConvArgs& a, hipStream_t s) {
  int cp, cinp, kp;
  if (vipe_conv_packed_dims(a.Cout, a.Cin, a.KH, a.KW, &cp, &cinp, &kp) != VIPE_OK) return VIPE_EINVAL;
  a.Cout_pad = cp;
  a.Cin_pad = cinp;
  a.nsteps = kp / 64;
  const int64_t M = (int64_t)a.B * a.H * a.W;
  if (M == 0) return VIPE_OK;
  const bool small = a.Cin == 4;
  const int gx = (int)((M + BNP - 1) / BNP);
  const bool sq13 = !small && a.KH == a.KW && (a.KH == 1 || a.KH == 3);
  const bool off32 = (int64_t)a.B * a.H * a.W < (1ll << 31);
  const bool aligned = a.W % HALO_TW == 0 && a.H % HALO_TH == 0;
  const bool halo = sq13 && aligned && off32;
  const bool flat = sq13 && !aligned && off32 && flat_geometry(a, a.KH == 3 ? 1 : 0);
  if (needs_tile_kernel(a) && !halo && !flat) return VIPE_EUNSUPPORTED;
  if (a.epi == EPI_GLO && a.KH == 1 && a.KW == 1 && a.Cin == 128 && a.Cout == 128 && cp == 128 && a.split >= a.Cin &&
      a.x0_ctot % 8 == 0 && a.x0_coff % 8 == 0 && a.net == a.x0 && a.net_ctot == a.x0_ctot && a.net_coff == a.x0_coff &&
      a.extra == nullptr) {
    static std::atomic<uint64_t> seen{0};
    allow_lds(conv1x1_glo_kernel, seen, GLO_LDS);
    conv1x1_glo_kernel<<<dim3((unsigned)(a.B * ((a.H * a.W + 255) / 256))), 512, GLO_LDS, s>>>(a);
    return vipe_launch_status();
  }
  if (halo) {
    const int rc = launch_halo_family<false>(a, cp, M, s);
    if (rc != VIPE_EUNSUPPORTED || needs_tile_kernel(a)) return rc;
  } else if (flat) {
    const int rc = launch_halo_family<true>(a, cp, M, s);
    if (rc != VIPE_EUNSUPPORTED || needs_tile_kernel(a)) return rc;
  }
  if (small && a.KH == 7 && a.KW == 7 && cp % 128 == 0 && kp == 256 && a.epi == EPI_PLAIN && a.extra == nullptr &&
      (int64_t)a.B * a.H * a.W < (1ll << 31)) {
    const int gy = cp / 128;
    if (aligned) {
      static std::atomic<uint64_t> seen{0};
      allow_lds(conv7x7_c4_kernel<false>, seen, C7_LDS);
      conv7x7_c4_kernel<false><<<dim3((int)(M / (HALO_TH * HALO_TW)) * gy), 512, C7_LDS, s>>>(a, gy);
      return vipe_launch_status();
    }
    flat_geometry(a, 3);
    const size_t need = C7_WBYTES + (size_t)(256 + 6 * a.f_wp + 6) * 8;
    if (need <= MAX_LDS && a.f_hwp < (1 << 23) && a.f_wp >= 2) {
      static std::atomic<uint64_t> seen{0};
      allow_lds(conv7x7_c4_kernel<true>, seen, MAX_LDS);
      const size_t lds = need > (size_t)(256 * 136 * 2) ? need : (size_t)(256 * 136 * 2);
      conv7x7_c4_kernel<true><<<dim3(a.B * a.f_tiles * gy), 512, lds, s>>>(a, gy);
      return vipe_launch_status();
    }
  }
  const bool glds = !small && a.KH * a.KW <= 32;
  static std::atomic<uint64_t> s1{0}, s2{0}, s3{0};
  allow_lds(conv_mfma_kernel<128, 2, 2, false>, s1, 65536);
  allow_lds(conv_mfma_kernel<128, 2, 2, true>, s2, 65536);
  allow_lds(conv_mfma_glds_kernel<128, 2, 2>, s3, 65536);
  if (cp >= 128) {
    const size_t lds = 2 * (128 + BNP) * 128;
    const int gy = cp / 128;
    if (small) conv_mfma_kernel<128, 2, 2, true><<<dim3(gx, gy), 256, lds, s>>>(a);
    else if (glds) conv_mfma_glds_kernel<128, 2, 2><<<dim3(gx * gy), 256, lds, s>>>(a, gy);
    else conv_mfma_kernel<128, 2, 2, false><<<dim3(gx, gy), 256, lds, s>>>(a);
  } else if (cp == 64) {
    const size_t lds = 2 * (64 + BNP) * 128;
    if (small) return VIPE_EUNSUPPORTED;
    if (glds) conv_mfma_glds_kernel<64, 1, 4><<<dim3(gx), 256, lds, s>>>(a, 1);
    else conv_mfma_kernel<64, 1, 4, false><<<dim3(gx, 1), 256, lds, s>>>(a);
  } else {
    const size_t lds = 2 * (32 + BNP) * 128;
    if (small) return VIPE_EUNSUPPORTED;
    if (glds) conv_mfma_glds_kernel<32, 1, 4><<<dim3(gx), 256, lds, s>>>(a, 1);
    else conv_mfma_kernel<32, 1, 4, false><<<dim3(gx, 1), 256, lds, s>>>(a);
  }
  return vipe_launch_status();
}

}

extern "C" {

VIPE_EXPORT int vipe_conv2d_nhwc_f16(const void* d_x, const void* d_w_packed, const float* d_bias,
                                     const float* d_extra, void* d_y, int B, int H, int W, int Cin, int cin_total,
                                     int cin_off, int Cout, int cout_total, int cout_off, int KH, int KW, int act,
                                     void* stream) {
  VIPE_CHECK_ARG(d_x && d_w_packed && d_bias && d_y);
  VIPE_CHECK_ARG(B >= 0 && H > 0 && W > 0 && Cin > 0 && Cout > 0 && (KH & 1) && (KW & 1));
  VIPE_CHECK_ARG((Cin == 4 || Cin % 8 == 0) && cin_total % 4 == 0 && cin_off % 4 == 0 && cout_total % 4 == 0 &&
                 cout_off % 4 == 0);
  VIPE_CHECK_ARG(Cin == 4 || (cin_total % 8 == 0 && cin_off % 8 == 0));
  VIPE_CHECK_ARG(act >= 0 && act <= 3);
  ConvArgs a = {};
  a.x0 = (const half_t*)d_x; a.x0_ctot = cin_total; a.x0_coff = cin_off;
  a.x1 = a.x0; a.x1_ctot = cin_total; a.x1_coff = cin_off; a.split = Cin;
  a.w = (const half_t*)d_w_packed; a.bias = d_bias; a.extra = d_extra; a.extra_stride = Cout; a.extra_off = 0;
  a.y = (half_t*)d_y; a.y_ctot = cout_total; a.y_coff = cout_off;
  a.B = B; a.H = H; a.W = W; a.Cin = Cin; a.Cout = Cout; a.KH = KH; a.KW = KW;
  a.act = act; a.epi = EPI_PLAIN;
  return launch_conv(a, as_stream(stream));
}

VIPE_EXPORT int vipe_conv2d_fused(const void* d_x0, int x0_ctot, int x0_coff, const void* d_x1, int x1_ctot,
                                  int x1_coff, int split, const void* d_w_packed, const float* d_bias,
                                  const float* d_extra, int extra_stride, int extra_off, void* d_y, int y_ctot,
                                  int y_coff, void* d_y2, int y2_ctot, int y2_coff, const void* d_net, int net_ctot,
                                  int net_coff, const void* d_z, float* d_fout, const void* d_accinit, int ai_ctot,
                                  int ai_coff, int B, int H, int W, int Cin, int Cout, int KH, int KW, int act, int mode,
                                  void* stream) {
  VIPE_CHECK_ARG(d_x0 && d_w_packed && d_bias);
  VIPE_CHECK_ARG(!d_accinit || (ai_ctot % 4 == 0 && ai_coff % 4 == 0 && ai_coff + Cout <= ai_ctot));
  VIPE_CHECK_ARG(B >= 0 && H > 0 && W > 0 && Cin > 0 && Cout > 0 && (KH & 1) && (KW & 1));
  if (Cin == 4) {
    VIPE_CHECK_ARG(split >= Cin && x0_ctot % 4 == 0 && x0_coff % 4 == 0);
  } else {
    VIPE_CHECK_ARG(Cin % 8 == 0 && x0_ctot % 8 == 0 && x0_coff % 8 == 0);
    VIPE_CHECK_ARG(split >= Cin || (split % 64 == 0 && d_x1 && x1_ctot % 8 == 0 && x1_coff % 8 == 0));
  }
  const int ai_f32 = (mode & VIPE_CONV_ACCINIT_F32) != 0;
  mode &= ~VIPE_CONV_ACCINIT_F32;
  VIPE_CHECK_ARG(mode >= EPI_PLAIN && mode <= EPI_PARTIAL);
  if (mode == EPI_PARTIAL) VIPE_CHECK_ARG(d_fout && y_ctot % 4 == 0 && y_coff % 4 == 0 && y_coff + Cout <= y_ctot && !d_extra);
  if (mode == EPI_PLAIN) VIPE_CHECK_ARG(d_y && y_ctot % 4 == 0 && y_coff % 4 == 0);
  if (mode == EPI_GLO) VIPE_CHECK_ARG(d_net && d_fout);
  if (mode == EPI_ZR) VIPE_CHECK_ARG(d_y && d_y2 && d_net && Cout == 256);
  if (mode == EPI_Q) VIPE_CHECK_ARG(d_y && d_net && d_z && Cout == 128);
  if (mode == EPI_HEADS) VIPE_CHECK_ARG(d_fout && Cout == 4);
  if (mode == EPI_ETA) VIPE_CHECK_ARG(d_fout && Cout == 1);
  ConvArgs a = {};
  a.x0 = (const half_t*)d_x0; a.x0_ctot = x0_ctot; a.x0_coff = x0_coff;
  a.x1 = (const half_t*)(d_x1 ? d_x1 : d_x0); a.x1_ctot = d_x1 ? x1_ctot : x0_ctot; a.x1_coff = d_x1 ? x1_coff : x0_coff;
  a.split = split > Cin ? Cin : split;
  a.w = (const half_t*)d_w_packed; a.bias = d_bias; a.extra = d_extra; a.extra_stride = extra_stride; a.extra_off = extra_off;
  a.y = (half_t*)d_y; a.y_ctot = y_ctot; a.y_coff = y_coff;
  a.y2 = (half_t*)d_y2; a.y2_ctot = y2_ctot; a.y2_coff = y2_coff;
  a.net = (const half_t*)d_net; a.net_ctot = net_ctot; a.net_coff = net_coff;
  a.zbuf = (const half_t*)d_z; a.fout = d_fout;
  a.accinit = (const half_t*)d_accinit; a.ai_ctot = ai_ctot; a.ai_coff = ai_coff; a.ai_f32 = ai_f32;
  a.B = B; a.H = H; a.W = W; a.Cin = Cin; a.Cout = Cout; a.KH = KH; a.KW = KW;
  a.act = act; a.epi = mode;
  return launch_conv(a, as_stream(stream));
}

}
```

### vipe_amd/ext/droid_net_ext.py

```python

import ctypes

import torch

from .._lib import DTYPE_CODE, check, check_gpu_contig, lib, ptr, require, stream_ptr


def corr_index_forward(volume, coords, radius):
    check_gpu_contig(volume, coords)
    require(volume.dim() == 5 and coords.dim() == 4 and coords.dtype == torch.float32, "bad corr_index_forward inputs")
    require(volume.dtype in DTYPE_CODE, "volume must be half/float/double")
    B, h1, w1, h2, w2 = volume.shape
    require(tuple(coords.shape) == (B, 2, h1, w1), "coords must be [B,2,h1,w1]")
    rd = 2 * radius + 1
    corr = torch.empty((B, rd, rd, h1, w1), dtype=volume.dtype, device=volume.device)
    check(lib().vipe_corr_index_forward(ptr(volume), ptr(coords), ptr(corr), B, h1, w1, h2, w2, radius,
                                        DTYPE_CODE[volume.dtype], stream_ptr(volume)), "corr_index_forward")
    return [corr]


def corr_index_backward(volume, coords, corr_grad, radius):
    check_gpu_contig(volume, coords, corr_grad)
    B, h1, w1, h2, w2 = volume.shape
    require(corr_grad.dtype == volume.dtype, "corr_grad dtype must match volume")
    grad = torch.empty_like(volume)
    check(lib().vipe_corr_index_backward(ptr(coords), ptr(corr_grad), ptr(grad), B, h1, w1, h2, w2, radius,
                                         DTYPE_CODE[volume.dtype], stream_ptr(volume)), "corr_index_backward")
    return [grad]


def altcorr_forward(fmap1, fmap2, coords, radius):
    check_gpu_contig(fmap1, fmap2, coords)
    require(fmap1.dtype == fmap2.dtype and fmap1.dtype in (torch.float16, torch.float32), "fmaps must be half/float")
    require(coords.dtype == torch.float32 and coords.dim() == 5, "coords must be [B,N,H1,W1,2] float32")
    B, H1, W1, C = fmap1.shape
    _, H2, W2, _ = fmap2.shape
    N = coords.shape[1]
    rd = 2 * radius + 1
    corr = torch.empty((B, N, rd * rd, H1, W1), dtype=fmap1.dtype, device=fmap1.device)
    check(lib().vipe_altcorr_forward(ptr(fmap1), ptr(fmap2), ptr(coords), ptr(corr), B, H1, W1, H2, W2, N, C,
                                     radius, DTYPE_CODE[fmap1.dtype], stream_ptr(fmap1)), "altcorr_forward")
    return [corr]


def altcorr_backward(fmap1, fmap2, coords, corr_grad, radius):
    check_gpu_contig(fmap1, fmap2, coords, corr_grad)
    require(fmap1.dtype == torch.float32 and fmap2.dtype == torch.float32, "altcorr_backward is float32 only")
    B, H1, W1, C = fmap1.shape
    _, H2, W2, _ = fmap2.shape
    N = coords.shape[1]
    g1 = torch.zeros_like(fmap1)
    g2 = torch.zeros_like(fmap2)
    check(lib().vipe_altcorr_backward(ptr(fmap1), ptr(fmap2), ptr(coords), ptr(corr_grad), ptr(g1), ptr(g2), B, H1,
                                      W1, H2, W2, N, C, radius, stream_ptr(fmap1)), "altcorr_backward")
    return [g1, g2, torch.zeros_like(coords)]




def corr_volume(fmap1, fmap2):
    E, C, h, w = fmap1.shape
    if fmap1.is_cuda and fmap1.dtype == fmap2.dtype and fused_build_covers(C, h, w, 1, fmap1.dtype):
        return corr_pyramid_build(fmap1, fmap2, 1)[0].reshape(E, h * w, h * w)
    check_gpu_contig(fmap1, fmap2)
    require(fmap1.dtype == fmap2.dtype and fmap1.dtype in DTYPE_CODE, "fmaps must be half/float/double of one dtype")
    vol = torch.empty((E, h * w, h * w), dtype=fmap1.dtype, device=fmap1.device)
    check(lib().vipe_corr_volume(ptr(fmap1), ptr(fmap2), ptr(vol), E, C, h * w, DTYPE_CODE[fmap1.dtype], stream_ptr(fmap1)),
          "corr_volume")
    return vol


REFERENCE, BLOCKED = 0, 1


def blocked_dims(h, w):
    d = (ctypes.c_int * 6)()
    check(lib().vipe_corr_blocked_dims(h, w, ctypes.cast(d, ctypes.c_void_p)), "corr_blocked_dims")
    return tuple(int(x) for x in d[:5]) + (bool(d[5]),)


def fused_build_covers(C, h, w, num_levels, dtype=torch.float16):
    return dtype == torch.float16 and C == 128 and num_levels <= 4 and (h >> (num_levels - 1)) > 0 and (w >> (num_levels - 1)) > 0


def pyramid_level_shapes(n, h, w, num_levels, layout):
    shapes = [(n, h, w, h >> i, w >> i) for i in range(num_levels)]
    if layout == BLOCKED:
        G, S, R, w2p, w3p, direct = blocked_dims(h, w)
        shapes[0] = (n, G, S * R, 64, 4, 4, 8)
        if num_levels > 1:
            shapes[1] = (n, G, S * R // 2, 64, 2, 4, 8)
        if not direct:
            if num_levels > 2:
                shapes[2] = (n, G * 64, R, w2p)
            if num_levels > 3:
                shapes[3] = (n, G * 64, R // 2, w3p)
    return shapes


def pyramid_to_reference(levels, h, w):
    out = list(levels)
    if not len(levels) or levels[0].dim() != 7:
        return out
    G, S, R, w2p, w3p, direct = blocked_dims(h, w)
    P = h * w
    for i in range(min(2, len(levels))):
        lv = levels[i]
        n, T, Ri = lv.shape[0], lv.shape[4], R >> i
        x = lv.reshape(n, G, S, Ri, 64, T, 4, 8).permute(0, 1, 4, 3, 6, 2, 5, 7).reshape(n, G * 64, Ri * 4, S * T * 8)
        out[i] = x[:, :P, :h >> i, :w >> i].reshape(n, h, w, h >> i, w >> i).contiguous()
    if not direct:
        for i in range(2, len(levels)):
            out[i] = levels[i][:, :P, :h >> i, :w >> i].reshape(levels[i].shape[0], h, w, h >> i, w >> i).contiguous()
    return out


def pyramid_to_blocked(levels, h, w):
    G, S, R, w2p, w3p, direct = blocked_dims(h, w)
    P = h * w
    out = list(levels)
    n = levels[0].shape[0]
    for i in range(len(levels)):
        lv = levels[i].reshape(n, P, h >> i, w >> i)
        if i < 2:
            T, Ri = 4 >> i, R >> i
            x = lv.new_zeros((n, G * 64, Ri * 4, S * T * 8))
            x[:, :P, :h >> i, :w >> i] = lv
            x = x.reshape(n, G, 64, Ri, 4, S, T, 8).permute(0, 1, 5, 3, 2, 6, 4, 7)
            out[i] = x.reshape(n, G, S * Ri, 64, T, 4, 8).contiguous()
        elif not direct:
            x = lv.new_zeros((n, G * 64, R >> (i - 2), w2p if i == 2 else w3p))
            x[:, :P, :h >> i, :w >> i] = lv
            out[i] = x
    return out


def _level_ptrs(levels):
    return (ctypes.c_void_p * len(levels))(*[lv.data_ptr() for lv in levels])


def corr_prep(fmaps):
    check_gpu_contig(fmaps)
    n, C, h, w = fmaps.shape
    per = int(lib().vipe_corr_prep_halves(C, h, w))
    require(per > 0 and fmaps.dtype == torch.float16, "corr_prep: fp16 maps with 128 channels")
    prep = torch.empty((n, per), dtype=torch.float16, device=fmaps.device)
    check(lib().vipe_corr_prep(ptr(fmaps), ptr(prep), n, C, h, w, stream_ptr(fmaps)), "corr_prep")
    return prep


def corr_pyramid_build(fmap1, fmap2, num_levels=4, layout=REFERENCE):
    E, C, h, w = fmap1.shape
    if fmap1.dtype == fmap2.dtype and fmap1.is_cuda and fused_build_covers(C, h, w, num_levels, fmap1.dtype):
        check_gpu_contig(fmap1, fmap2)
        if blocked_dims(h, w)[5] and layout == REFERENCE:
            levels = [torch.empty((E, h, w, h >> i, w >> i), dtype=torch.float16, device=fmap1.device)
                      for i in range(num_levels)]
            check(lib().vipe_corr_pyramid_build(ptr(fmap1), ptr(fmap2), _level_ptrs(levels), E, C, h, w, num_levels,
                                                stream_ptr(fmap1)), "corr_pyramid_build")
            return levels
        idx = torch.arange(2 * E, device=fmap1.device)
        levels = corr_pyramid_build_indexed(torch.cat([fmap1, fmap2], 0), idx[:E], idx[E:], num_levels=num_levels,
                                            frame_range=(0, 2 * E))
        return levels if layout == BLOCKED else [lv.contiguous() for lv in pyramid_to_reference(levels, h, w)]
    require(layout == REFERENCE, "the blocked layout is the fp16 / 128-channel kernel's")
    check_gpu_contig(fmap1, fmap2)
    vol = corr_volume(fmap1, fmap2)
    levels = [vol.view(E, h, w, h, w)]
    hl, wl = h, w
    for i in range(1, num_levels):
        nxt = torch.empty((E, h, w, hl >> 1, wl >> 1), dtype=vol.dtype, device=vol.device)
        check(lib().vipe_avg_pool2x2(ptr(levels[-1]), ptr(nxt), E * h * w, hl, wl, DTYPE_CODE[vol.dtype], stream_ptr(vol)),
              "avg_pool2x2")
        levels.append(nxt)
        hl, wl = hl >> 1, wl >> 1
    return levels


def corr_pyramid_build_indexed(fmaps, idx1, idx2, levels=None, slots=None, layout=BLOCKED, num_levels=4, frame_range=None):
    n, C, h, w = fmaps.shape
    E = int(idx1.shape[0])
    require(fused_build_covers(C, h, w, num_levels, fmaps.dtype) and fmaps.is_cuda,
            "corr_pyramid_build_indexed: fp16 maps on the device, C == 128, h, w >= 2^(levels-1)")
    check_gpu_contig(fmaps, idx1, idx2)
    require(idx1.dtype == torch.int64 and idx2.dtype == torch.int64 and idx2.shape[0] == E, "idx1 / idx2: int64 [E]")
    direct = blocked_dims(h, w)[5]
    require(direct or layout == BLOCKED, "the reference layout needs w % 64 == 0 and h % 8 == 0 (use corr_pyramid_build)")
    if levels is None:
        levels = [torch.empty(s, dtype=torch.float16, device=fmaps.device)
                  for s in pyramid_level_shapes(E, h, w, num_levels, layout)]
    else:
        want = pyramid_level_shapes(levels[0].shape[0], h, w, num_levels, layout)
        require(len(levels) == num_levels and all(tuple(lv.shape) == s and lv.is_contiguous() for lv, s in zip(levels, want)),
                "level buffers do not match the layout")
    if slots is not None:
        check_gpu_contig(slots)
        require(slots.dtype == torch.int32 and slots.shape[0] == E, "slots: int32 [E]")
    if E == 0:
        return levels
    sl = ptr(slots) if slots is not None else None
    if direct:
        check(lib().vipe_corr_pyramid_build_indexed(ptr(fmaps), ptr(idx1), ptr(idx2), sl, _level_ptrs(levels), E, C, h, w,
                                                    num_levels, layout, stream_ptr(fmaps)), "corr_pyramid_build_indexed")
        return levels
    if frame_range is None:
        both = torch.cat([idx1, idx2])
        frame_range = (int(both.min().item()), int(both.max().item()) + 1)
    lo, hi = max(0, int(frame_range[0])), min(n, int(frame_range[1]))
    require(hi > lo, "corr_pyramid_build_indexed: empty frame range")
    prep = corr_prep(fmaps[lo:hi])
    check(lib().vipe_corr_pyramid_build_prepared(ptr(prep), lo, hi - lo, ptr(idx1), ptr(idx2), sl, _level_ptrs(levels), E, C, h, w,
                                                 num_levels, stream_ptr(fmaps)), "corr_pyramid_build_prepared")
    return levels


def corr_pyramid_lookup(levels, coords, radius=3):
    check_gpu_contig(coords, *levels)
    require(coords.dtype == torch.float32, "coords must be float32")
    E, h1, w1, h2, w2 = levels[0].shape
    L = len(levels)
    for i, lv in enumerate(levels):
        require(tuple(lv.shape) == (E, h1, w1, h2 >> i, w2 >> i) and lv.dtype == levels[0].dtype, "bad pyramid level")
    require(tuple(coords.shape) == (E, h1, w1, 2), "coords must be [E,h1,w1,2]")
    rd = 2 * radius + 1
    out = torch.empty((E, L * rd * rd, h1, w1), dtype=levels[0].dtype, device=coords.device)
    arr = (ctypes.c_void_p * L)(*[lv.data_ptr() for lv in levels])
    check(lib().vipe_corr_pyramid_lookup(ctypes.cast(arr, ctypes.c_void_p), ptr(coords), ptr(out), E, h1, w1, h2, w2,
                                         L, radius, DTYPE_CODE[levels[0].dtype], stream_ptr(coords)),
          "corr_pyramid_lookup")
    return out


def corr_pyramid_lookup_nhwc(levels, coords, radius=3, channel_stride=200):
    check_gpu_contig(coords, *levels)
    require(coords.dtype == torch.float32, "coords must be float32")
    E, h1, w1, h2, w2 = levels[0].shape
    L = len(levels)
    require(tuple(coords.shape) == (E, h1, w1, 2), "coords must be [E,h1,w1,2]")
    out = torch.empty((E, h1, w1, channel_stride), dtype=levels[0].dtype, device=coords.device)
    arr = (ctypes.c_void_p * L)(*[lv.data_ptr() for lv in levels])
    check(lib().vipe_corr_pyramid_lookup_nhwc(ctypes.cast(arr, ctypes.c_void_p), ptr(coords), ptr(out), E, h1, w1, h2,
                                              w2, L, radius, DTYPE_CODE[levels[0].dtype], channel_stride,
                                              stream_ptr(coords)), "corr_pyramid_lookup_nhwc")
    return out


def corr_lookup_conv1x1(levels, coords, w_packed, bias, out, out_coff=0, cout=128, act="relu", slots=None, grid=None):
    check_gpu_contig(coords, out, *levels)
    require(len(levels) == 4 and levels[0].dtype == torch.float16 and coords.dtype == torch.float32, "fp16 4-level pyramid")
    layout = BLOCKED if levels[0].dim() == 7 else REFERENCE
    cap = levels[2].shape[0]
    if levels[2].dim() == 5:
        h1, w1 = levels[2].shape[1:3]
        h2, w2 = levels[2].shape[3] << 2, levels[2].shape[4] << 2
    else:
        require(grid is not None, "a padded blocked store needs grid=(h, w)")
        h1, w1 = h2, w2 = int(grid[0]), int(grid[1])
    E = cap if slots is None else int(slots.shape[0])
    if slots is not None:
        check_gpu_contig(slots)
        require(slots.dtype == torch.int32 and E <= cap, "slots must be int32 [E], E <= pool capacity")
    require(tuple(coords.shape) == (E, h1, w1, 2) and tuple(out.shape[:3]) == (E, h1, w1) and out.dtype == torch.float16,
            "bad coords / out shape")
    arr = (ctypes.c_void_p * 4)(*[lv.data_ptr() for lv in levels])
    check(lib().vipe_corr_lookup_conv1x1(ctypes.cast(arr, ctypes.c_void_p), ptr(coords), ptr(w_packed), ptr(bias), ptr(out),
                                         out.shape[-1], out_coff, E, h1, w1, h2, w2, cout, {"none": 0, "relu": 1}[act],
                                         ptr(slots) if slots is not None else None, layout, stream_ptr(coords)),
          "corr_lookup_conv1x1")
    return out


def cvx_upsample(data, mask, rows=None, out=None, mask_layout="nhwc"):
    if not (data.is_cuda and mask.is_cuda):
        raise NotImplementedError("cvx_upsample: device tensors only (vipe_convex_upsample is a HIP kernel)")
    require(mask_layout in ("nhwc", "nchw"), "mask_layout must be 'nhwc' or 'nchw'")
    if mask_layout == "nchw":
        if mask.dim() == 5:
            mask = mask.reshape(-1, *mask.shape[2:])
        require(mask.dim() == 4 and mask.shape[1] == 576, "nchw mask must be [N,576,h,w]")
        mask = mask.permute(0, 2, 3, 1).contiguous()
    require(data.dim() == 4 and data.dtype == torch.float32, "data must be [R,h,w,C] float32")
    require(mask.dim() == 4 and mask.shape[3] == 576 and mask.dtype in (torch.float16, torch.float32),
            "mask must be [N,h,w,576] half/float")
    R, h, w, C = data.shape
    N = int(mask.shape[0])
    require(tuple(mask.shape[1:3]) == (h, w), "mask and data grids differ")
    if out is None:
        out = torch.zeros((R, 8 * h, 8 * w, C), dtype=torch.float32, device=data.device)
    require(tuple(out.shape) == (R, 8 * h, 8 * w, C) and out.dtype == torch.float32, "out must be [R,8h,8w,C] float32")
    check_gpu_contig(data, mask, out)
    if rows is not None:
        check_gpu_contig(rows)
        require(rows.dtype == torch.int64 and tuple(rows.shape) == (N,), "rows must be int64 [N]")
    else:
        require(N <= R, "more mask rows than data rows")
    check(lib().vipe_convex_upsample(ptr(mask), DTYPE_CODE[mask.dtype], ptr(data), ptr(out), ptr(rows), N, R, h, w, C,
                                     stream_ptr(data)), "convex_upsample")
    return out
```

Measured before the change: 261.8.

## Split last partial wave of 3x3 halo conv into half-width tiles

```diff
diff --git a/include/vipe_amd.h b/include/vipe_amd.h
--- a/include/vipe_amd.h
+++ b/include/vipe_amd.h
@@ -266,6 +266,8 @@
                       const void* d_accinit, int ai_ctot, int ai_coff, int B, int H, int W, int Cin, int Cout, int KH,
                       int KW, int act, int mode, void* stream);
 
+int vipe_conv_tail_policy(int mode, int slots);
+
 typedef struct {
   const void *corr0_w, *corr2_w, *flow0_w, *flow2_w, *gw_w, *zr_w, *q_w, *zr_s_w, *q_s_w, *heads0_w, *heads2_w, *agg2_w, *eta_w;
   const void *zr_n_w, *zr_x_w;
diff --git a/scratch/conv_tail_sweep.py b/scratch/conv_tail_sweep.py
--- /dev/null
+++ b/scratch/conv_tail_sweep.py
@@ -0,0 +1,90 @@
+import argparse
+import json
+import sys
+
+sys.path.insert(0, ".")
+import torch
+
+from oracle import conv_epilogue_cases as cases
+from vipe_amd._lib import check, lib, ptr, stream_ptr
+from vipe_amd.ext import droid_net_ext
+from vipe_amd.slam.update_engine import _Packed
+
+ap = argparse.ArgumentParser()
+ap.add_argument("--policies", default="off,forced")
+ap.add_argument("--slots", type=int, default=0)
+ap.add_argument("--grid", type=int, nargs=2, default=(48, 64))
+ap.add_argument("--edges", default="8,16,24,32,40,43,48,53,59,64,69,75,80,85,138,276")
+ap.add_argument("--layers", default="plain_corr2,q_ctx,zr_staged,zr_ctx,plain_heads0")
+ap.add_argument("--reps", type=int, default=20)
+ap.add_argument("--out", default=None)
+args = ap.parse_args()
+dev = torch.device("cuda:0")
+H, W = args.grid
+slots = args.slots or 2 * torch.cuda.get_device_properties(dev).multi_processor_count
+ACT = {"none": 0, "relu": 1, "sigmoid": 2, "tanh": 3}
+CH = {"net": 128, "xbuf": 320, "rnet": 128, "z": 128, "c1": 128, "pgate": 384, "pzr": 256}
+out = open(args.out, "w") if args.out else None
+torch.manual_seed(0)
+
+
+def launcher(name, E):
+    L = cases.LAUNCHES[name]
+    w, b = cases.weights(name)
+    pk = _Packed(w, b, dev)
+    bufs = {}
+
+    def buf(n):
+        if n is not None and n not in bufs:
+            t = torch.randn(E, H, W, CH[n], device=dev) * 0.5
+            bufs[n] = t if n == "pzr" else t.half()
+        return bufs.get(n)
+
+    x0, x1 = buf(L.x0[0]), buf(L.x1[0] if L.x1 else None)
+    init, net, z = buf(L.init[0] if L.init else None), buf(L.net), buf(L.z)
+    extra = torch.randn(E, 384, device=dev) * 0.1 if L.extra_off is not None else None
+    y = torch.empty(E, H, W, L.y[0], dtype=torch.float16, device=dev)
+    y2 = torch.empty(E, H, W, L.y2[0], dtype=torch.float16, device=dev) if L.y2 else None
+    mode = cases.MODE[L.mode] | (0x100 if init is not None and init.dtype == torch.float32 else 0)
+    pitch = lambda t: 0 if t is None else t.shape[-1]
+
+    def run():
+        check(lib().vipe_conv2d_fused(
+            ptr(x0), pitch(x0), L.x0[1], ptr(x1), pitch(x1), L.x1[1] if L.x1 else 0, L.split, ptr(pk.packed), ptr(pk.bias),
+            ptr(extra), pitch(extra), L.extra_off or 0, ptr(y), L.y[0], L.y[1], ptr(y2), L.y2[0] if L.y2 else 0,
+            L.y2[1] if L.y2 else 0, ptr(net), pitch(net), 0, ptr(z), None, ptr(init), pitch(init), L.init[1] if L.init else 0,
+            E, H, W, L.cin, L.cout, 3, 3, ACT[L.act], mode, stream_ptr(x0)), name)
+    return run, L
+
+
+for name in args.layers.split(","):
+    for E in [int(e) for e in args.edges.split(",")]:
+        run, L = launcher(name, E)
+        tiles = (H // 4) * (W // 64) if H % 4 == 0 and W % 64 == 0 else (H * (W + 1) + 255) // 256
+        n = E * tiles * ((L.cout + 127) // 128)
+        rec = {"layer": name, "E": E, "grid": [H, W], "workgroups": n, "slots": slots, "rounds": round(n / slots, 3),
+               "tail": n % slots}
+        for pol in args.policies.split(","):
+            droid_net_ext.conv_tail_policy(pol, slots if pol == "forced" else 0)
+            for _ in range(5):
+                run()
+            torch.cuda.synchronize()
+            e0, e1 = torch.cuda.Event(enable_timing=True), torch.cuda.Event(enable_timing=True)
+            best = []
+            for _ in range(3):
+                e0.record()
+                for _ in range(args.reps):
+                    run()
+                e1.record()
+                torch.cuda.synchronize()
+                best.append(e0.elapsed_time(e1) / args.reps * 1e3)
+            best.sort()
+            rec[pol + "_us"] = round(best[1], 1)
+            rec[pol + "_spread_us"] = round(best[2] - best[0], 1)
+            rec[pol + "_split_launches"] = droid_net_ext.conv_tail_policy("auto")
+        line = json.dumps(rec)
+        print(line, flush=True)
+        if out:
+            out.write(line + "\n")
+            out.flush()
+droid_net_ext.conv_tail_policy("auto")
diff --git a/vipe_amd/csrc/conv_halo32_body.inc b/vipe_amd/csrc/conv_halo32_body.inc
--- /dev/null
+++ b/vipe_amd/csrc/conv_halo32_body.inc
@@ -0,0 +1,378 @@
+  constexpr int MI = BMC >= 128 ? 4 : 2, NJ = BMC == 32 ? 2 : 4;
+  constexpr int BP = HALO_TH * HALO_TW;
+  constexpr int WSTAGE = BMC * 64;
+  extern __shared__ __align__(16) unsigned char lds[];
+
+  const int tid = threadIdx.x, lane = tid & 63, wave = __builtin_amdgcn_readfirstlane(tid >> 6);
+  const int wm = BMC == 32 ? 0 : (wave >> 2), wn = wave & 3;
+  const int pxh = BMC == 32 ? (wave >> 2) * 32 : 0;
+  const int tile = L / gy, cout0 = (L % gy) * BMC;
+  const int xsegs = a.W / HALO_TW, tiles_per_img = FLAT ? a.f_tiles : (a.H / HALO_TH) * xsegs;
+  const int e = tile / tiles_per_img, trem = tile % tiles_per_img;
+  const int y0 = (trem / xsegs) * HALO_TH, x0 = (trem % xsegs) * HALO_TW;
+  const int q0 = trem * BP;
+  const int pitch = FLAT ? a.f_wp : HALO_PITCH;
+  const int xbytes = FLAT ? a.f_xbytes : H32_XBYTES;
+  const int npieces = FLAT ? a.f_pieces : H32_PIECES;
+  auto pix_of = [&](int pl) -> int64_t {
+    if constexpr (FLAT) return flat_pixel(q0 + pl, e, a.H, a.W, a.f_wp, a.f_hwp, a.f_magic);
+    else return ((int64_t)(e * a.H + y0 + (pl >> 6))) * a.W + x0 + (pl & 63);
+  };
+  const int cs32 = a.Cin_pad / H32_BK, cs64 = a.Cin_pad / 64;
+  const int r16 = lane >> 2, sl = lane & 3;
+
+  const unsigned ldsW_a = lds_address(lds), ldsX_a = ldsW_a + 3 * WSTAGE;
+  const unsigned sink_a = ldsX_a + 2 * xbytes;
+  const unsigned char* ldsW = lds;
+  const unsigned char* ldsX = lds + 3 * WSTAGE;
+  const half_t* zp = reinterpret_cast<const half_t*>(g_zero_page);
+
+  constexpr int WPIECES = BMC / 16;
+  const bool wreal = wave < WPIECES;
+  const int wrow = (wave % WPIECES) * 16 + r16;
+  const unsigned woff = (unsigned)(wrow * 64 + ((sl ^ swzf(wrow)) << 3)) * 2u;
+  const unsigned wdst = ldsW_a + (wave % WPIECES) * 1024;
+  int xpix[FLAT ? 1 : H32_XP];
+  const int xk = (sl ^ swzf(r16)) * 8;
+  if constexpr (!FLAT) {
+#pragma unroll
+    for (int i = 0; i < H32_XP; ++i) {
+      const int pce = wave + 8 * i;
+      const int r = pce * 16 + r16;
+      const int hy = r / HALO_PITCH, hx = r % HALO_PITCH;
+      const int y = y0 + hy - 1, x = x0 + hx - 1;
+      const bool ok = pce < H32_PIECES && r < HALO_ROWS && y >= 0 && y < a.H && x >= 0 && x < a.W;
+      xpix[i] = ok ? (e * a.H + y) * a.W + x : -1;
+    }
+  }
+  auto piece_used = [&](int i) {
+    const int pce = wave + 8 * i;
+    if constexpr (FLAT) return pce < npieces && (KS == 3 || (pce >= a.f_p1lo && pce <= a.f_p1hi));
+    else return pce < H32_PIECES && (KS == 3 || (pce >= 4 && pce <= 20));
+  };
+  auto issueX = [&](int c, int i, int buf) {
+    const int c0 = c * H32_BK;
+    const bool s0 = c0 < a.split;
+    const int ctot = s0 ? a.x0_ctot : a.x1_ctot;
+    const int cb = (s0 ? a.x0_coff : a.x1_coff - a.split) + c0;
+    int xp;
+    if constexpr (FLAT) xp = flat_pixel(q0 - pitch - 1 + (wave + 8 * i) * 16 + r16, e, a.H, a.W, a.f_wp, a.f_hwp, a.f_magic);
+    else xp = xpix[i];
+    const bool ok = xp >= 0 && (c0 + xk < a.Cin);
+    const uint64_t off = ((uint64_t)(unsigned)xp * (unsigned)ctot + (unsigned)(cb + xk)) * 2u;
+    const char* src = reinterpret_cast<const char*>(s0 ? a.x0 : a.x1) + off;
+    glds16(ok ? (const void*)src : (const void*)zp, ldsX_a + buf * xbytes + (wave + 8 * i) * 1024);
+  };
+  auto wsrc = [&](int tap, int c) {
+    return a.w + ((int64_t)(tap * cs64 + (c >> 1)) * a.Cout_pad + cout0) * BK + (c & 1) * H32_BK;
+  };
+  auto issueW = [&](const half_t* wb, int slot) {
+    if (wreal) glds16_off(wb, woff, wdst + slot * WSTAGE);
+    else glds16(zp, sink_a);
+  };
+  const uint64_t zp64 = uniform64((uint64_t)zp);
+  const uint64_t wbase = uniform64((uint64_t)(a.w + (int64_t)cout0 * BK));
+  const unsigned tstride = (unsigned)cs64 * (unsigned)a.Cout_pad * BK * 2u;
+  const unsigned sink_u = __builtin_amdgcn_readfirstlane(sink_a), wdst_u = __builtin_amdgcn_readfirstlane(wdst);
+  const unsigned ldsX_u = __builtin_amdgcn_readfirstlane(ldsX_a + wave * 1024);
+  auto issueW2 = [&](int tap, int c, int slot, bool more_) {
+    const unsigned off = (unsigned)tap * tstride + ((unsigned)(c >> 1) * (unsigned)a.Cout_pad * BK + (unsigned)(c & 1) * H32_BK) * 2u;
+    const bool on = more_ && wreal;
+    dma16s(on ? wbase + off : zp64, on ? woff : 0u, on ? wdst_u + slot * WSTAGE : sink_u);
+  };
+  auto issueX2 = [&](int c, int i, int buf, bool on) {
+    const int c0 = c * H32_BK;
+    const bool s0 = c0 < a.split;
+    const int ctot = s0 ? a.x0_ctot : a.x1_ctot;
+    const int cb = (s0 ? a.x0_coff : a.x1_coff - a.split) + c0;
+    int xp;
+    if constexpr (FLAT) xp = flat_pixel(q0 - pitch - 1 + (wave + 8 * i) * 16 + r16, e, a.H, a.W, a.f_wp, a.f_hwp, a.f_magic);
+    else xp = xpix[i];
+    const bool ok = on && xp >= 0 && (c0 + xk < a.Cin);
+    const uint64_t off = ((uint64_t)(unsigned)xp * (unsigned)ctot + (unsigned)(cb + xk)) * 2u;
+    const uint64_t base = (uint64_t)(s0 ? a.x0 : a.x1);
+    dma16v(ok ? base + off : zp64, on ? ldsX_u + buf * xbytes + i * 8192 : sink_u);
+  };
+
+  float4v acc16[MI][NJ];
+#pragma unroll
+  for (int i = 0; i < MI; ++i)
+#pragma unroll
+    for (int j = 0; j < NJ; ++j) acc16[i][j] = float4v{0.0f, 0.0f, 0.0f, 0.0f};
+  if constexpr (BMC >= 64) {
+    if (a.accinit) {
+#pragma unroll
+      for (int j = 0; j < NJ; ++j) {
+        const int64_t m = pix_of(wn * 64 + j * 16 + (lane & 15));
+        if (FLAT && m < 0) continue;
+#pragma unroll
+        for (int i = 0; i < MI; ++i) {
+          const int cg = cout0 + wm * (MI * 16) + i * 16 + 4 * (lane >> 4);
+          if constexpr (VAR == 1) {
+            const float4 v = *reinterpret_cast<const float4*>(reinterpret_cast<const float*>(a.accinit) + m * a.ai_ctot +
+                                                              a.ai_coff + cg);
+            acc16[i][j] = float4v{v.x, v.y, v.z, v.w};
+          } else {
+            const half4 v = *reinterpret_cast<const half4*>(a.accinit + m * a.ai_ctot + a.ai_coff + cg);
+            acc16[i][j] = float4v{(float)v[0], (float)v[1], (float)v[2], (float)v[3]};
+          }
+        }
+      }
+    }
+  }
+
+  const int l16 = lane & 15, lk = lane >> 4;
+  const int wa0 = swz32(wm * MI * 16 + l16, lk);
+  const int Rl0 = (FLAT ? wn * HALO_TW : wn * HALO_PITCH) + pxh + l16;
+  auto mma_step = [&](const unsigned char* bw, const unsigned char* bx, int Rl, int dy, int dx) {
+    const int rb = Rl + (dy + 1) * pitch + (dx + 1);
+    const int xa0 = swz32(rb, lk);
+    half8 wf[MI];
+#pragma unroll
+    for (int i = 0; i < MI; ++i) wf[i] = *reinterpret_cast<const half8*>(bw + (wa0 + i * 1024));
+#pragma unroll
+    for (int j = 0; j < NJ; ++j) {
+      const half8 xf = *reinterpret_cast<const half8*>(bx + (xa0 + j * 1024));
+#pragma unroll
+      for (int i = 0; i < MI; ++i)
+        acc16[i][j] = __builtin_amdgcn_mfma_f32_16x16x32_f16(wf[i], xf, acc16[i][j], 0, 0, 0);
+    }
+  };
+
+  auto load_frags = [&](const unsigned char* bw, const unsigned char* bx, int Rl, int dy, int dx, half8 (&wf)[MI], half8 (&xf)[NJ]) {
+    const int xa0 = swz32(Rl + (dy + 1) * pitch + (dx + 1), lk);
+#pragma unroll
+    for (int i = 0; i < MI; ++i) wf[i] = *reinterpret_cast<const half8*>(bw + (wa0 + i * 1024));
+#pragma unroll
+    for (int j = 0; j < NJ; ++j) xf[j] = *reinterpret_cast<const half8*>(bx + (xa0 + j * 1024));
+  };
+  auto mma_frags = [&](const half8 (&wf)[MI], const half8 (&xf)[NJ]) {
+#pragma unroll
+    for (int j = 0; j < NJ; ++j)
+#pragma unroll
+      for (int i = 0; i < MI; ++i) acc16[i][j] = __builtin_amdgcn_mfma_f32_16x16x32_f16(wf[i], xf[j], acc16[i][j], 0, 0, 0);
+  };
+
+#pragma unroll
+  for (int i = 0; i < H32_XP; ++i)
+    if (piece_used(i)) issueX(0, i, 0);
+  issueW(wsrc(0, 0), 0);
+  if constexpr (KS == 3) issueW(wsrc(1, 0), 1);
+  asm volatile("s_waitcnt vmcnt(0)" ::: "memory");
+  __syncthreads();
+
+  if constexpr (KS == 3) {
+    for (int c = 0; c < cs32; ++c) {
+      const unsigned char* bx = ldsX + (c & 1) * xbytes;
+      const bool more = c + 1 < cs32;
+      int Rl = Rl0;
+      asm volatile("" : "+v"(Rl));
+      auto tap_step = [&](auto TAPC) {
+        constexpr int TAP = decltype(TAPC)::value;
+        constexpr int T2 = TAP + 2;
+        half8 wf[MI], xf[NJ];
+        load_frags(ldsW + (TAP % 3) * WSTAGE, bx, Rl, TAP / 3 - 1, TAP % 3 - 1, wf, xf);
+        if constexpr (T2 < 9) issueW2(T2, c, T2 % 3, true);
+        else issueW2(T2 - 9, c + 1, T2 % 3, more);
+        if constexpr (TAP < H32_XP) issueX2(c + 1, TAP, (c + 1) & 1, more && piece_used(TAP));
+        mma_frags(wf, xf);
+        if constexpr (TAP == 0 || TAP == 4) asm volatile("s_waitcnt vmcnt(2)" ::: "memory");
+        else if constexpr (TAP < 4) asm volatile("s_waitcnt vmcnt(3)" ::: "memory");
+        else asm volatile("s_waitcnt vmcnt(1)" ::: "memory");
+        __syncthreads();
+      };
+      tap_step(std::integral_constant<int, 0>{});
+      tap_step(std::integral_constant<int, 1>{});
+      tap_step(std::integral_constant<int, 2>{});
+      tap_step(std::integral_constant<int, 3>{});
+      tap_step(std::integral_constant<int, 4>{});
+      tap_step(std::integral_constant<int, 5>{});
+      tap_step(std::integral_constant<int, 6>{});
+      tap_step(std::integral_constant<int, 7>{});
+      tap_step(std::integral_constant<int, 8>{});
+    }
+  } else {
+    for (int c = 0; c < cs32; ++c) {
+      const unsigned char* bx = ldsX + (c & 1) * xbytes;
+      if (c + 1 < cs32) {
+        issueW(wsrc(0, c + 1), (c + 1) & 1);
+#pragma unroll
+        for (int i = 0; i < H32_XP; ++i)
+          if (piece_used(i)) issueX(c + 1, i, (c + 1) & 1);
+      }
+      mma_step(ldsW + (c & 1) * WSTAGE, bx, Rl0, 0, 0);
+      asm volatile("s_waitcnt vmcnt(0)" ::: "memory");
+      __syncthreads();
+    }
+  }
+  asm volatile("s_waitcnt vmcnt(0)" ::: "memory");
+  __syncthreads();
+
+  constexpr int CPP = BMC / 8;
+  constexpr int NIT = BP * CPP / 512, PSTEP = 512 / CPP;
+  const int ch = (tid % CPP) * 8, co = cout0 + ch, pl0 = tid / CPP;
+  if constexpr (BMC >= 64) {
+    if constexpr (VAR == 2) {
+      {
+#pragma unroll
+        for (int j = 0; j < NJ; ++j) {
+          const int64_t m = pix_of(wn * 64 + j * 16 + l16);
+          if (FLAT && m < 0) continue;
+#pragma unroll
+          for (int i = 0; i < MI; ++i) {
+            const int cg = cout0 + wm * (MI * 16) + i * 16 + 4 * lk;
+            if (cg + 4 <= a.Cout)
+              *reinterpret_cast<float4*>(a.fout + m * a.y_ctot + a.y_coff + cg) =
+                  make_float4(acc16[i][j][0], acc16[i][j][1], acc16[i][j][2], acc16[i][j][3]);
+          }
+        }
+        return;
+      }
+    }
+    constexpr int PITCH = BMC + 8;
+    half_t* stage = reinterpret_cast<half_t*>(lds);
+    auto stage_all = [&](auto ACTC) {
+      constexpr int ACT = decltype(ACTC)::value;
+      auto put = [&](int cl, int pl, float4 b, float v0, float v1, float v2, float v3) {
+        half4 h;
+        h[0] = (half_t)act_apply(v0 + b.x, ACT);
+        h[1] = (half_t)act_apply(v1 + b.y, ACT);
+        h[2] = (half_t)act_apply(v2 + b.z, ACT);
+        h[3] = (half_t)act_apply(v3 + b.w, ACT);
+        *reinterpret_cast<half4*>(stage + pl * PITCH + cl) = h;
+      };
+      auto bias4 = [&](int cl) {
+        const int cg = cout0 + cl;
+        float4 b = *reinterpret_cast<const float4*>(a.bias + cg);
+        if (a.extra && cg + 4 <= a.Cout) {
+          const float4 x = *reinterpret_cast<const float4*>(a.extra + (int64_t)e * a.extra_stride + a.extra_off + cg);
+          b.x += x.x; b.y += x.y; b.z += x.z; b.w += x.w;
+        }
+        return b;
+      };
+#pragma unroll
+      for (int i = 0; i < MI; ++i) {
+        const int cl = wm * (MI * 16) + i * 16 + 4 * lk;
+        const float4 b = bias4(cl);
+#pragma unroll
+        for (int j = 0; j < NJ; ++j)
+          put(cl, wn * 64 + j * 16 + l16, b, acc16[i][j][0], acc16[i][j][1], acc16[i][j][2], acc16[i][j][3]);
+      }
+    };
+    const int actsel = a.epi == EPI_PLAIN ? a.act : (a.epi == EPI_Q ? VIPE_ACT_TANH : VIPE_ACT_SIGMOID);
+    if (actsel == VIPE_ACT_RELU) stage_all(std::integral_constant<int, VIPE_ACT_RELU>{});
+    else if (actsel == VIPE_ACT_SIGMOID) stage_all(std::integral_constant<int, VIPE_ACT_SIGMOID>{});
+    else if (actsel == VIPE_ACT_TANH) stage_all(std::integral_constant<int, VIPE_ACT_TANH>{});
+    else stage_all(std::integral_constant<int, VIPE_ACT_NONE>{});
+    const bool want_net = a.epi == EPI_GLO || a.epi == EPI_Q || (a.epi == EPI_ZR && co >= 128);
+    const bool want_z = a.epi == EPI_Q;
+    half8 nvv[NIT], zvv[NIT];
+    {
+      const int cn = a.epi == EPI_ZR ? co - 128 : co;
+#pragma unroll
+      for (int it = 0; it < NIT; ++it) {
+        const int64_t m = pix_of(pl0 + PSTEP * it);
+        if (FLAT && m < 0) continue;
+        if (want_net) nvv[it] = *reinterpret_cast<const half8*>(a.net + m * a.net_ctot + a.net_coff + cn);
+        if (want_z) zvv[it] = *reinterpret_cast<const half8*>(a.zbuf + m * 128 + co);
+      }
+    }
+    __syncthreads();
+    float gsum[8] = {0, 0, 0, 0, 0, 0, 0, 0};
+#pragma unroll
+    for (int it = 0; it < NIT; ++it) {
+      const int pl = pl0 + PSTEP * it;
+      const int64_t m = pix_of(pl);
+      if (FLAT && m < 0) continue;
+      const half8 sv = *reinterpret_cast<const half8*>(stage + pl * PITCH + ch);
+      half8 o = sv;
+      half_t* dst = nullptr;
+      if (a.epi == EPI_PLAIN) {
+        dst = a.y + m * a.y_ctot + a.y_coff + co;
+      } else if (a.epi == EPI_GLO) {
+#pragma unroll
+        for (int q = 0; q < 8; ++q) gsum[q] += (float)sv[q] * (float)nvv[it][q];
+      } else if (a.epi == EPI_ZR) {
+        if (co < 128) {
+          dst = a.y + m * a.y_ctot + a.y_coff + co;
+        } else {
+#pragma unroll
+          for (int q = 0; q < 8; ++q) o[q] = (half_t)((float)sv[q] * (float)nvv[it][q]);
+          dst = a.y2 + m * a.y2_ctot + a.y2_coff + co - 128;
+        }
+      } else if (a.epi == EPI_Q) {
+#pragma unroll
+        for (int q = 0; q < 8; ++q) {
+          const float z = (float)zvv[it][q];
+          o[q] = (half_t)((1.0f - z) * (float)nvv[it][q] + z * (float)sv[q]);
+        }
+        dst = a.y + m * a.y_ctot + a.y_coff + co;
+      }
+      if (dst) {
+        if (co + 8 <= a.Cout) {
+          *reinterpret_cast<half8*>(dst) = o;
+        } else {
+          for (int q = 0; q < 8 && co + q < a.Cout; ++q) dst[q] = o[q];
+        }
+      }
+    }
+    if (a.epi == EPI_GLO) {
+      float* red = reinterpret_cast<float*>(lds);
+      __syncthreads();
+#pragma unroll
+      for (int q = 0; q < 8; ++q) red[(tid / CPP) * (BMC + 1) + ch + q] = gsum[q];
+      __syncthreads();
+      if (tid < BMC) {
+        float t = 0.0f;
+        for (int r = 0; r < 512 / CPP; ++r) t += red[r * (BMC + 1) + tid];
+        if (cout0 + tid < a.Cout) atomicAdd(a.fout + (int64_t)e * a.Cout + cout0 + tid, t);
+      }
+    }
+  } else {
+    constexpr int PITCH = BMC + 4;
+    float* stage = reinterpret_cast<float*>(lds);
+#pragma unroll
+    for (int i = 0; i < MI; ++i)
+#pragma unroll
+      for (int j = 0; j < NJ; ++j)
+        *reinterpret_cast<float4*>(stage + (wn * 64 + pxh + j * 16 + l16) * PITCH + i * 16 + 4 * lk) =
+            make_float4(acc16[i][j][0], acc16[i][j][1], acc16[i][j][2], acc16[i][j][3]);
+    __syncthreads();
+    float bv[8];
+#pragma unroll
+    for (int q = 0; q < 8; ++q) {
+      bv[q] = a.bias[co + q];
+      if (a.extra && co + q < a.Cout) bv[q] += a.extra[(int64_t)e * a.extra_stride + a.extra_off + co + q];
+    }
+#pragma unroll
+    for (int it = 0; it < NIT; ++it) {
+      const int pl = pl0 + PSTEP * it;
+      const int64_t m = pix_of(pl);
+      if (FLAT && m < 0) continue;
+      const float4 v0 = *reinterpret_cast<const float4*>(stage + pl * PITCH + ch);
+      const float4 v1 = *reinterpret_cast<const float4*>(stage + pl * PITCH + ch + 4);
+      const float v[8] = {v0.x + bv[0], v0.y + bv[1], v0.z + bv[2], v0.w + bv[3],
+                          v1.x + bv[4], v1.y + bv[5], v1.z + bv[6], v1.w + bv[7]};
+      if (a.epi == EPI_HEADS) {
+        if (ch == 0)
+          *reinterpret_cast<float4*>(a.fout + m * 4) =
+              make_float4((float)(half_t)v[0], (float)(half_t)v[1], (float)(half_t)act_apply(v[2], VIPE_ACT_SIGMOID),
+                          (float)(half_t)act_apply(v[3], VIPE_ACT_SIGMOID));
+      } else if (a.epi == EPI_ETA) {
+        if (ch == 0) {
+          const float sp = v[0] > 20.0f ? v[0] : log1pf(__expf(v[0]));
+          a.fout[m] = 0.01f * (float)(half_t)sp;
+        }
+      } else {
+        half_t* dst = a.y + m * a.y_ctot + a.y_coff + co;
+        half8 o;
+#pragma unroll
+        for (int q = 0; q < 8; ++q) o[q] = (half_t)act_apply(v[q], a.act);
+        if (co + 8 <= a.Cout) {
+          *reinterpret_cast<half8*>(dst) = o;
+        } else {
+          for (int q = 0; q < 8 && co + q < a.Cout; ++q) dst[q] = o[q];
+        }
+      }
+    }
+  }
diff --git a/vipe_amd/csrc/conv_mfma.hip b/vipe_amd/csrc/conv_mfma.hip
--- a/vipe_amd/csrc/conv_mfma.hip
+++ b/vipe_amd/csrc/conv_mfma.hip
@@ -381,385 +381,21 @@
 template <int BMC, int KS, bool M16, int VAR = 0, bool FLAT = false>
 __global__ __launch_bounds__(512) __attribute__((amdgpu_waves_per_eu(4, 4))) void conv_halo32_kernel(ConvArgs a, int gy) {
   static_assert(M16, "only the 16x16x32 form exists");
-  constexpr int MI = BMC >= 128 ? 4 : 2, NJ = BMC == 32 ? 2 : 4;
-  constexpr int BP = HALO_TH * HALO_TW;
-  constexpr int WSTAGE = BMC * 64;
-  extern __shared__ __align__(16) unsigned char lds[];
-
-  const int tid = threadIdx.x, lane = tid & 63, wave = __builtin_amdgcn_readfirstlane(tid >> 6);
-  const int wm = BMC == 32 ? 0 : (wave >> 2), wn = wave & 3;
-  const int pxh = BMC == 32 ? (wave >> 2) * 32 : 0;
   const int L = xcd_remap(blockIdx.x, gridDim.x);
-  const int tile = L / gy, cout0 = (L % gy) * BMC;
-  const int xsegs = a.W / HALO_TW, tiles_per_img = FLAT ? a.f_tiles : (a.H / HALO_TH) * xsegs;
-  const int e = tile / tiles_per_img, trem = tile % tiles_per_img;
-  const int y0 = (trem / xsegs) * HALO_TH, x0 = (trem % xsegs) * HALO_TW;
-  const int q0 = trem * BP;
-  const int pitch = FLAT ? a.f_wp : HALO_PITCH;
-  const int xbytes = FLAT ? a.f_xbytes : H32_XBYTES;
-  const int npieces = FLAT ? a.f_pieces : H32_PIECES;
-  auto pix_of = [&](int pl) -> int64_t {
-    if constexpr (FLAT) return flat_pixel(q0 + pl, e, a.H, a.W, a.f_wp, a.f_hwp, a.f_magic);
-    else return ((int64_t)(e * a.H + y0 + (pl >> 6))) * a.W + x0 + (pl & 63);
-  };
-  const int cs32 = a.Cin_pad / H32_BK, cs64 = a.Cin_pad / 64;
-  const int r16 = lane >> 2, sl = lane & 3;
-
-  const unsigned ldsW_a = lds_address(lds), ldsX_a = ldsW_a + 3 * WSTAGE;
-  const unsigned sink_a = ldsX_a + 2 * xbytes;
-  const unsigned char* ldsW = lds;
-  const unsigned char* ldsX = lds + 3 * WSTAGE;
-  const half_t* zp = reinterpret_cast<const half_t*>(g_zero_page);
-
-  constexpr int WPIECES = BMC / 16;
-  const bool wreal = wave < WPIECES;
-  const int wrow = (wave % WPIECES) * 16 + r16;
-  const unsigned woff = (unsigned)(wrow * 64 + ((sl ^ swzf(wrow)) << 3)) * 2u;
-  const unsigned wdst = ldsW_a + (wave % WPIECES) * 1024;
-  int xpix[FLAT ? 1 : H32_XP];
-  const int xk = (sl ^ swzf(r16)) * 8;
-  if constexpr (!FLAT) {
-#pragma unroll
-    for (int i = 0; i < H32_XP; ++i) {
-      const int pce = wave + 8 * i;
-      const int r = pce * 16 + r16;
-      const int hy = r / HALO_PITCH, hx = r % HALO_PITCH;
-      const int y = y0 + hy - 1, x = x0 + hx - 1;
-      const bool ok = pce < H32_PIECES && r < HALO_ROWS && y >= 0 && y < a.H && x >= 0 && x < a.W;
-      xpix[i] = ok ? (e * a.H + y) * a.W + x : -1;
-    }
-  }
-  auto piece_used = [&](int i) {
-    const int pce = wave + 8 * i;
-    if constexpr (FLAT) return pce < npieces && (KS == 3 || (pce >= a.f_p1lo && pce <= a.f_p1hi));
-    else return pce < H32_PIECES && (KS == 3 || (pce >= 4 && pce <= 20));
-  };
-  auto issueX = [&](int c, int i, int buf) {
-    const int c0 = c * H32_BK;
-    const bool s0 = c0 < a.split;
-    const int ctot = s0 ? a.x0_ctot : a.x1_ctot;
-    const int cb = (s0 ? a.x0_coff : a.x1_coff - a.split) + c0;
-    int xp;
-    if constexpr (FLAT) xp = flat_pixel(q0 - pitch - 1 + (wave + 8 * i) * 16 + r16, e, a.H, a.W, a.f_wp, a.f_hwp, a.f_magic);
-    else xp = xpix[i];
-    const bool ok = xp >= 0 && (c0 + xk < a.Cin);
-    const uint64_t off = ((uint64_t)(unsigned)xp * (unsigned)ctot + (unsigned)(cb + xk)) * 2u;
-    const char* src = reinterpret_cast<const char*>(s0 ? a.x0 : a.x1) + off;
-    glds16(ok ? (const void*)src : (const void*)zp, ldsX_a + buf * xbytes + (wave + 8 * i) * 1024);
-  };
-  auto wsrc = [&](int tap, int c) {
-    return a.w + ((int64_t)(tap * cs64 + (c >> 1)) * a.Cout_pad + cout0) * BK + (c & 1) * H32_BK;
-  };
-  auto issueW = [&](const half_t* wb, int slot) {
-    if (wreal) glds16_off(wb, woff, wdst + slot * WSTAGE);
-    else glds16(zp, sink_a);
-  };
-  const uint64_t zp64 = uniform64((uint64_t)zp);
-  const uint64_t wbase = uniform64((uint64_t)(a.w + (int64_t)cout0 * BK));
-  const unsigned tstride = (unsigned)cs64 * (unsigned)a.Cout_pad * BK * 2u;
-  const unsigned sink_u = __builtin_amdgcn_readfirstlane(sink_a), wdst_u = __builtin_amdgcn_readfirstlane(wdst);
-  const unsigned ldsX_u = __builtin_amdgcn_readfirstlane(ldsX_a + wave * 1024);
-  auto issueW2 = [&](int tap, int c, int slot, bool more_) {
-    const unsigned off = (unsigned)tap * tstride + ((unsigned)(c >> 1) * (unsigned)a.Cout_pad * BK + (unsigned)(c & 1) * H32_BK) * 2u;
-    const bool on = more_ && wreal;
-    dma16s(on ? wbase + off : zp64, on ? woff : 0u, on ? wdst_u + slot * WSTAGE : sink_u);
-  };
-  auto issueX2 = [&](int c, int i, int buf, bool on) {
-    const int c0 = c * H32_BK;
-    const bool s0 = c0 < a.split;
-    const int ctot = s0 ? a.x0_ctot : a.x1_ctot;
-    const int cb = (s0 ? a.x0_coff : a.x1_coff - a.split) + c0;
-    int xp;
-    if constexpr (FLAT) xp = flat_pixel(q0 - pitch - 1 + (wave + 8 * i) * 16 + r16, e, a.H, a.W, a.f_wp, a.f_hwp, a.f_magic);
-    else xp = xpix[i];
-    const bool ok = on && xp >= 0 && (c0 + xk < a.Cin);
-    const uint64_t off = ((uint64_t)(unsigned)xp * (unsigned)ctot + (unsigned)(cb + xk)) * 2u;
-    const uint64_t base = (uint64_t)(s0 ? a.x0 : a.x1);
-    dma16v(ok ? base + off : zp64, on ? ldsX_u + buf * xbytes + i * 8192 : sink_u);
-  };
-
-  float4v acc16[MI][NJ];
-#pragma unroll
-  for (int i = 0; i < MI; ++i)
-#pragma unroll
-    for (int j = 0; j < NJ; ++j) acc16[i][j] = float4v{0.0f, 0.0f, 0.0f, 0.0f};
-  if constexpr (BMC >= 64) {
-    if (a.accinit) {
-#pragma unroll
-      for (int j = 0; j < NJ; ++j) {
-        const int64_t m = pix_of(wn * 64 + j * 16 + (lane & 15));
-        if (FLAT && m < 0) continue;
-#pragma unroll
-        for (int i = 0; i < MI; ++i) {
-          const int cg = cout0 + wm * (MI * 16) + i * 16 + 4 * (lane >> 4);
-          if constexpr (VAR == 1) {
-            const float4 v = *reinterpret_cast<const float4*>(reinterpret_cast<const float*>(a.accinit) + m * a.ai_ctot +
-                                                              a.ai_coff + cg);
-            acc16[i][j] = float4v{v.x, v.y, v.z, v.w};
-          } else {
-            const half4 v = *reinterpret_cast<const half4*>(a.accinit + m * a.ai_ctot + a.ai_coff + cg);
-            acc16[i][j] = float4v{(float)v[0], (float)v[1], (float)v[2], (float)v[3]};
-          }
-        }
-      }
-    }
-  }
-
-  const int l16 = lane & 15, lk = lane >> 4;
-  const int wa0 = swz32(wm * MI * 16 + l16, lk);
-  const int Rl0 = (FLAT ? wn * HALO_TW : wn * HALO_PITCH) + pxh + l16;
-  auto mma_step = [&](const unsigned char* bw, const unsigned char* bx, int Rl, int dy, int dx) {
-    const int rb = Rl + (dy + 1) * pitch + (dx + 1);
-    const int xa0 = swz32(rb, lk);
-    half8 wf[MI];
-#pragma unroll
-    for (int i = 0; i < MI; ++i) wf[i] = *reinterpret_cast<const half8*>(bw + (wa0 + i * 1024));
-#pragma unroll
-    for (int j = 0; j < NJ; ++j) {
-      const half8 xf = *reinterpret_cast<const half8*>(bx + (xa0 + j * 1024));
-#pragma unroll
-      for (int i = 0; i < MI; ++i)
-        acc16[i][j] = __builtin_amdgcn_mfma_f32_16x16x32_f16(wf[i], xf, acc16[i][j], 0, 0, 0);
-    }
-  };
-
-  auto load_frags = [&](const unsigned char* bw, const unsigned char* bx, int Rl, int dy, int dx, half8 (&wf)[MI], half8 (&xf)[NJ]) {
-    const int xa0 = swz32(Rl + (dy + 1) * pitch + (dx + 1), lk);
-#pragma unroll
-    for (int i = 0; i < MI; ++i) wf[i] = *reinterpret_cast<const half8*>(bw + (wa0 + i * 1024));
-#pragma unroll
-    for (int j = 0; j < NJ; ++j) xf[j] = *reinterpret_cast<const half8*>(bx + (xa0 + j * 1024));
-  };
-  auto mma_frags = [&](const half8 (&wf)[MI], const half8 (&xf)[NJ]) {
-#pragma unroll
-    for (int j = 0; j < NJ; ++j)
-#pragma unroll
-      for (int i = 0; i < MI; ++i) acc16[i][j] = __builtin_amdgcn_mfma_f32_16x16x32_f16(wf[i], xf[j], acc16[i][j], 0, 0, 0);
-  };
-
-#pragma unroll
-  for (int i = 0; i < H32_XP; ++i)
-    if (piece_used(i)) issueX(0, i, 0);
-  issueW(wsrc(0, 0), 0);
-  if constexpr (KS == 3) issueW(wsrc(1, 0), 1);
-  asm volatile("s_waitcnt vmcnt(0)" ::: "memory");
-  __syncthreads();
-
-  if constexpr (KS == 3) {
-    for (int c = 0; c < cs32; ++c) {
-      const unsigned char* bx = ldsX + (c & 1) * xbytes;
-      const bool more = c + 1 < cs32;
-      int Rl = Rl0;
-      asm volatile("" : "+v"(Rl));
-      auto tap_step = [&](auto TAPC) {
-        constexpr int TAP = decltype(TAPC)::value;
-        constexpr int T2 = TAP + 2;
-        half8 wf[MI], xf[NJ];
-        load_frags(ldsW + (TAP % 3) * WSTAGE, bx, Rl, TAP / 3 - 1, TAP % 3 - 1, wf, xf);
-        if constexpr (T2 < 9) issueW2(T2, c, T2 % 3, true);
-        else issueW2(T2 - 9, c + 1, T2 % 3, more);
-        if constexpr (TAP < H32_XP) issueX2(c + 1, TAP, (c + 1) & 1, more && piece_used(TAP));
-        mma_frags(wf, xf);
-        if constexpr (TAP == 0 || TAP == 4) asm volatile("s_waitcnt vmcnt(2)" ::: "memory");
-        else if constexpr (TAP < 4) asm volatile("s_waitcnt vmcnt(3)" ::: "memory");
-        else asm volatile("s_waitcnt vmcnt(1)" ::: "memory");
-        __syncthreads();
-      };
-      tap_step(std::integral_constant<int, 0>{});
-      tap_step(std::integral_constant<int, 1>{});
-      tap_step(std::integral_constant<int, 2>{});
-      tap_step(std::integral_constant<int, 3>{});
-      tap_step(std::integral_constant<int, 4>{});
-      tap_step(std::integral_constant<int, 5>{});
-      tap_step(std::integral_constant<int, 6>{});
-      tap_step(std::integral_constant<int, 7>{});
-      tap_step(std::integral_constant<int, 8>{});
-    }
-  } else {
-    for (int c = 0; c < cs32; ++c) {
-      const unsigned char* bx = ldsX + (c & 1) * xbytes;
-      if (c + 1 < cs32) {
-        issueW(wsrc(0, c + 1), (c + 1) & 1);
-#pragma unroll
-        for (int i = 0; i < H32_XP; ++i)
-          if (piece_used(i)) issueX(c + 1, i, (c + 1) & 1);
-      }
-      mma_step(ldsW + (c & 1) * WSTAGE, bx, Rl0, 0, 0);
-      asm volatile("s_waitcnt vmcnt(0)" ::: "memory");
-      __syncthreads();
-    }
-  }
-  asm volatile("s_waitcnt vmcnt(0)" ::: "memory");
-  __syncthreads();
-
-  constexpr int CPP = BMC / 8;
-  constexpr int NIT = BP * CPP / 512, PSTEP = 512 / CPP;
-  const int ch = (tid % CPP) * 8, co = cout0 + ch, pl0 = tid / CPP;
-  if constexpr (BMC >= 64) {
-    if constexpr (VAR == 2) {
-      {
-#pragma unroll
-        for (int j = 0; j < NJ; ++j) {
-          const int64_t m = pix_of(wn * 64 + j * 16 + l16);
-          if (FLAT && m < 0) continue;
-#pragma unroll
-          for (int i = 0; i < MI; ++i) {
-            const int cg = cout0 + wm * (MI * 16) + i * 16 + 4 * lk;
-            if (cg + 4 <= a.Cout)
-              *reinterpret_cast<float4*>(a.fout + m * a.y_ctot + a.y_coff + cg) =
-                  make_float4(acc16[i][j][0], acc16[i][j][1], acc16[i][j][2], acc16[i][j][3]);
-          }
-        }
-        return;
-      }
-    }
-    constexpr int PITCH = BMC + 8;
-    half_t* stage = reinterpret_cast<half_t*>(lds);
-    auto stage_all = [&](auto ACTC) {
-      constexpr int ACT = decltype(ACTC)::value;
-      auto put = [&](int cl, int pl, float4 b, float v0, float v1, float v2, float v3) {
-        half4 h;
-        h[0] = (half_t)act_apply(v0 + b.x, ACT);
-        h[1] = (half_t)act_apply(v1 + b.y, ACT);
-        h[2] = (half_t)act_apply(v2 + b.z, ACT);
-        h[3] = (half_t)act_apply(v3 + b.w, ACT);
-        *reinterpret_cast<half4*>(stage + pl * PITCH + cl) = h;
-      };
-      auto bias4 = [&](int cl) {
-        const int cg = cout0 + cl;
-        float4 b = *reinterpret_cast<const float4*>(a.bias + cg);
-        if (a.extra && cg + 4 <= a.Cout) {
-          const float4 x = *reinterpret_cast<const float4*>(a.extra + (int64_t)e * a.extra_stride + a.extra_off + cg);
-          b.x += x.x; b.y += x.y; b.z += x.z; b.w += x.w;
-        }
-        return b;
-      };
-#pragma unroll
-      for (int i = 0; i < MI; ++i) {
-        const int cl = wm * (MI * 16) + i * 16 + 4 * lk;
-        const float4 b = bias4(cl);
-#pragma unroll
-        for (int j = 0; j < NJ; ++j)
-          put(cl, wn * 64 + j * 16 + l16, b, acc16[i][j][0], acc16[i][j][1], acc16[i][j][2], acc16[i][j][3]);
-      }
-    };
-    const int actsel = a.epi == EPI_PLAIN ? a.act : (a.epi == EPI_Q ? VIPE_ACT_TANH : VIPE_ACT_SIGMOID);
-    if (actsel == VIPE_ACT_RELU) stage_all(std::integral_constant<int, VIPE_ACT_RELU>{});
-    else if (actsel == VIPE_ACT_SIGMOID) stage_all(std::integral_constant<int, VIPE_ACT_SIGMOID>{});
-    else if (actsel == VIPE_ACT_TANH) stage_all(std::integral_constant<int, VIPE_ACT_TANH>{});
-    else stage_all(std::integral_constant<int, VIPE_ACT_NONE>{});
-    const bool want_net = a.epi == EPI_GLO || a.epi == EPI_Q || (a.epi == EPI_ZR && co >= 128);
-    const bool want_z = a.epi == EPI_Q;
-    half8 nvv[NIT], zvv[NIT];
-    {
-      const int cn = a.epi == EPI_ZR ? co - 128 : co;
-#pragma unroll
-      for (int it = 0; it < NIT; ++it) {
-        const int64_t m = pix_of(pl0 + PSTEP * it);
-        if (FLAT && m < 0) continue;
-        if (want_net) nvv[it] = *reinterpret_cast<const half8*>(a.net + m * a.net_ctot + a.net_coff + cn);
-        if (want_z) zvv[it] = *reinterpret_cast<const half8*>(a.zbuf + m * 128 + co);
-      }
-    }
-    __syncthreads();
-    float gsum[8] = {0, 0, 0, 0, 0, 0, 0, 0};
-#pragma unroll
-    for (int it = 0; it < NIT; ++it) {
-      const int pl = pl0 + PSTEP * it;
-      const int64_t m = pix_of(pl);
-      if (FLAT && m < 0) continue;
-      const half8 sv = *reinterpret_cast<const half8*>(stage + pl * PITCH + ch);
-      half8 o = sv;
-      half_t* dst = nullptr;
-      if (a.epi == EPI_PLAIN) {
-        dst = a.y + m * a.y_ctot + a.y_coff + co;
-      } else if (a.epi == EPI_GLO) {
-#pragma unroll
-        for (int q = 0; q < 8; ++q) gsum[q] += (float)sv[q] * (float)nvv[it][q];
-      } else if (a.epi == EPI_ZR) {
-        if (co < 128) {
-          dst = a.y + m * a.y_ctot + a.y_coff + co;
-        } else {
-#pragma unroll
-          for (int q = 0; q < 8; ++q) o[q] = (half_t)((float)sv[q] * (float)nvv[it][q]);
-          dst = a.y2 + m * a.y2_ctot + a.y2_coff + co - 128;
-        }
-      } else if (a.epi == EPI_Q) {
-#pragma unroll
-        for (int q = 0; q < 8; ++q) {
-          const float z = (float)zvv[it][q];
-          o[q] = (half_t)((1.0f - z) * (float)nvv[it][q] + z * (float)sv[q]);
-        }
-        dst = a.y + m * a.y_ctot + a.y_coff + co;
-      }
-      if (dst) {
-        if (co + 8 <= a.Cout) {
-          *reinterpret_cast<half8*>(dst) = o;
-        } else {
-          for (int q = 0; q < 8 && co + q < a.Cout; ++q) dst[q] = o[q];
-        }
-      }
-    }
-    if (a.epi == EPI_GLO) {
-      float* red = reinterpret_cast<float*>(lds);
-      __syncthreads();
-#pragma unroll
-      for (int q = 0; q < 8; ++q) red[(tid / CPP) * (BMC + 1) + ch + q] = gsum[q];
-      __syncthreads();
-      if (tid < BMC) {
-        float t = 0.0f;
-        for (int r = 0; r < 512 / CPP; ++r) t += red[r * (BMC + 1) + tid];
-        if (cout0 + tid < a.Cout) atomicAdd(a.fout + (int64_t)e * a.Cout + cout0 + tid, t);
-      }
-    }
-  } else {
-    constexpr int PITCH = BMC + 4;
-    float* stage = reinterpret_cast<float*>(lds);
-#pragma unroll
-    for (int i = 0; i < MI; ++i)
-#pragma unroll
-      for (int j = 0; j < NJ; ++j)
-        *reinterpret_cast<float4*>(stage + (wn * 64 + pxh + j * 16 + l16) * PITCH + i * 16 + 4 * lk) =
-            make_float4(acc16[i][j][0], acc16[i][j][1], acc16[i][j][2], acc16[i][j][3]);
-    __syncthreads();
-    float bv[8];
-#pragma unroll
-    for (int q = 0; q < 8; ++q) {
-      bv[q] = a.bias[co + q];
-      if (a.extra && co + q < a.Cout) bv[q] += a.extra[(int64_t)e * a.extra_stride + a.extra_off + co + q];
-    }
-#pragma unroll
-    for (int it = 0; it < NIT; ++it) {
-      const int pl = pl0 + PSTEP * it;
-      const int64_t m = pix_of(pl);
-      if (FLAT && m < 0) continue;
-      const float4 v0 = *reinterpret_cast<const float4*>(stage + pl * PITCH + ch);
-      const float4 v1 = *reinterpret_cast<const float4*>(stage + pl * PITCH + ch + 4);
-      const float v[8] = {v0.x + bv[0], v0.y + bv[1], v0.z + bv[2], v0.w + bv[3],
-                          v1.x + bv[4], v1.y + bv[5], v1.z + bv[6], v1.w + bv[7]};
-      if (a.epi == EPI_HEADS) {
-        if (ch == 0)
-          *reinterpret_cast<float4*>(a.fout + m * 4) =
-              make_float4((float)(half_t)v[0], (float)(half_t)v[1], (float)(half_t)act_apply(v[2], VIPE_ACT_SIGMOID),
-                          (float)(half_t)act_apply(v[3], VIPE_ACT_SIGMOID));
-      } else if (a.epi == EPI_ETA) {
-        if (ch == 0) {
-          const float sp = v[0] > 20.0f ? v[0] : log1pf(__expf(v[0]));
-          a.fout[m] = 0.01f * (float)(half_t)sp;
-        }
-      } else {
-        half_t* dst = a.y + m * a.y_ctot + a.y_coff + co;
-        half8 o;
-#pragma unroll
-        for (int q = 0; q < 8; ++q) o[q] = (half_t)act_apply(v[q], a.act);
-        if (co + 8 <= a.Cout) {
-          *reinterpret_cast<half8*>(dst) = o;
-        } else {
-          for (int q = 0; q < 8 && co + q < a.Cout; ++q) dst[q] = o[q];
-        }
-      }
-    }
-  }
+#include "conv_halo32_body.inc"
+}
+
+template <int BMC, int KS, int VAR, bool FLAT>
+__device__ __forceinline__ void conv_halo32_body(const ConvArgs& a, int gy, const int L) {
+#include "conv_halo32_body.inc"
+}
+
+template <int KS, int VAR, bool FLAT>
+__global__ __launch_bounds__(512) __attribute__((amdgpu_waves_per_eu(4, 4))) void conv_halo32_tail_kernel(ConvArgs a, int gy,
+                                                                                                          int n_head) {
+  const int bid = (int)blockIdx.x;
+  if (bid < n_head) conv_halo32_body<128, KS, VAR, FLAT>(a, gy, xcd_remap(bid, n_head));
+  else conv_halo32_body<64, KS, VAR, FLAT>(a, 2 * gy, 2 * n_head + xcd_remap(bid - n_head, (int)gridDim.x - n_head));
 }
 
 constexpr int NRW_WBYTES = 9 * 1024;
@@ -1141,11 +777,49 @@
 
 inline bool needs_tile_kernel(const ConvArgs& a) { return a.accinit || a.epi == EPI_PARTIAL || a.ai_f32; }
 
+std::atomic<int> g_tail_mode{1};
+std::atomic<int> g_tail_slots{0};
+std::atomic<unsigned> g_tail_launches{0};
+constexpr int TAIL_MAX_NUM = 1, TAIL_MAX_DEN = 4;
+
+template <typename K>
+int device_slots(K kernel, size_t lds, std::atomic<uint64_t> (&cache)[64]) {
+  int d = 0;
+  (void)hipGetDevice(&d);
+  std::atomic<uint64_t>& c = cache[d & 63];
+  const uint64_t v = c.load(std::memory_order_acquire);
+  if ((v >> 32) == (uint64_t)lds + 1) return (int)(v & 0xffffffffu);
+  int cus = 0, per_cu = 0;
+  if (hipDeviceGetAttribute(&cus, hipDeviceAttributeMultiprocessorCount, d) != hipSuccess) cus = 0;
+  if (hipOccupancyMaxActiveBlocksPerMultiprocessor(&per_cu, kernel, 512, lds) != hipSuccess) per_cu = 0;
+  const int slots = cus > 0 && per_cu > 0 ? cus * per_cu : 0;
+  c.store((((uint64_t)lds + 1) << 32) | (unsigned)slots, std::memory_order_release);
+  return slots;
+}
+
 template <int BMC, int KS, int VAR, bool FLAT>
 int launch_halo32(const ConvArgs& a, int tiles, int gy, size_t lds, hipStream_t s) {
   static std::atomic<uint64_t> seen{0};
+  const int n = tiles * gy;
+  if constexpr (BMC == 128 && KS == 3) {
+    const int mode = a.epi == EPI_GLO ? 0 : g_tail_mode.load(std::memory_order_relaxed);
+    if (mode != 0) {
+      static std::atomic<uint64_t> seen_tail{0};
+      static std::atomic<uint64_t> slot_cache[64];
+      allow_lds(conv_halo32_tail_kernel<KS, VAR, FLAT>, seen_tail, FLAT ? MAX_LDS : lds);
+      const int slots = mode == 2 ? g_tail_slots.load(std::memory_order_relaxed)
+                                  : device_slots(conv_halo32_tail_kernel<KS, VAR, FLAT>, lds, slot_cache);
+      const int tail = slots > 0 ? n % slots : 0;
+      const bool gains = (int64_t)tail * TAIL_MAX_DEN <= (int64_t)slots * TAIL_MAX_NUM && (!FLAT || tail == n);
+      if (tail > 0 && (mode == 2 || gains)) {
+        g_tail_launches.fetch_add(1u, std::memory_order_relaxed);
+        conv_halo32_tail_kernel<KS, VAR, FLAT><<<dim3(n + tail), 512, lds, s>>>(a, gy, n - tail);
+        return vipe_launch_status();
+      }
+    }
+  }
   allow_lds(conv_halo32_kernel<BMC, KS, true, VAR, FLAT>, seen, FLAT ? MAX_LDS : lds);
-  conv_halo32_kernel<BMC, KS, true, VAR, FLAT><<<dim3(tiles * gy), 512, lds, s>>>(a, gy);
+  conv_halo32_kernel<BMC, KS, true, VAR, FLAT><<<dim3(n), 512, lds, s>>>(a, gy);
   return vipe_launch_status();
 }
 
@@ -1265,6 +939,13 @@
 
 extern "C" {
 
+VIPE_EXPORT int vipe_conv_tail_policy(int mode, int slots) {
+  VIPE_CHECK_ARG(mode >= 0 && mode <= 2 && (mode != 2 || slots > 0));
+  g_tail_slots.store(mode == 2 ? slots : 0, std::memory_order_relaxed);
+  g_tail_mode.store(mode, std::memory_order_relaxed);
+  return (int)(g_tail_launches.exchange(0u, std::memory_order_relaxed) & 0x7fffffffu);
+}
+
 VIPE_EXPORT int vipe_conv2d_nhwc_f16(const void* d_x, const void* d_w_packed, const float* d_bias,
                                      const float* d_extra, void* d_y, int B, int H, int W, int Cin, int cin_total,
                                      int cin_off, int Cout, int cout_total, int cout_off, int KH, int KW, int act,
diff --git a/vipe_amd/ext/droid_net_ext.py b/vipe_amd/ext/droid_net_ext.py
--- a/vipe_amd/ext/droid_net_ext.py
+++ b/vipe_amd/ext/droid_net_ext.py
@@ -270,6 +270,16 @@
     return out
 
 
+CONV_TAIL_POLICY = {"off": 0, "auto": 1, "forced": 2}
+
+
+def conv_tail_policy(mode="auto", slots=0):
+    code = lib().vipe_conv_tail_policy(CONV_TAIL_POLICY[mode], int(slots))
+    if code < 0:
+        check(code, "conv_tail_policy")
+    return code
+
+
 def cvx_upsample(data, mask, rows=None, out=None, mask_layout="nhwc"):
     if not (data.is_cuda and mask.is_cuda):
         raise NotImplementedError("cvx_upsample: device tensors only (vipe_convex_upsample is a HIP kernel)")
```

Result: no change. 260.9 (-0.3%).
